# LiWentomng/OrientedRepPoints

Hardware: NVIDIA H100
Metric: 1024x1024 tiles/sec (higher is better)
Workload: dtype f16x3

## Files before the change

include/orp_b200.h:

```cpp
#ifndef ORP_B200_H_
#define ORP_B200_H_

#include <stdint.h>

#ifdef __cplusplus
extern "C" {
#endif

#define ORP_OK 0
#define ORP_EINVAL (-1)
#define ORP_ECUDA (-2)
#define ORP_ENOGPU (-3)
#define ORP_EOVERFLOW (-4)

const char *orp_last_error(void);
int orp_version(void);
int orp_compiled_sm(void);
int64_t orp_launch_count(void);
void orp_reset_launch_count(void);


#define ORP_NMS_EXACT64 0
#define ORP_NMS_COMPAT32 1

#define ORP_UNION_NAN_KEEPS 0
#define ORP_UNION_GUARD 1
#define ORP_UNION_NAN_SUPPRESSES 2
#define ORP_UNION_NAN_SUPPRESSES_ALL 3

#define ORP_ORDER_INDEX_ASC 0
#define ORP_ORDER_SCORE_DESC 1

int orp_rnms(const float *dets, const int32_t *segments, int n, double iou_thr, int iou_mode,
             int union_mode, int order, int64_t *keep_out, int32_t *num_out, void *stream);

int orp_poly_nms_host(int *keep_out, int *num_out, const float *polys_host, int polys_num,
                      int polys_dim, float nms_overlap_thresh, int device_id);

typedef struct {
    int64_t pairs_total;
    int64_t pairs_aabb;
    int64_t pairs_clipped;
    int64_t pairs_fp64;
    int64_t edges;
    int64_t suppressing;
    int32_t overflow;
    int32_t rounds;
    int32_t n;
} orp_nms_stats;
int orp_rnms_last_stats(orp_nms_stats *out);

typedef struct {
    int32_t lazy;
    int32_t R;
    int32_t seg_limit;
    int32_t sweep_bits;
    int32_t no_sync;
    int32_t flags_out;
    int32_t union_mode, order, n;
    int64_t cap_first;
    int64_t cap_final;
    int32_t attempts;
} orp_rnms_plan;
int orp_rnms_last_plan(orp_rnms_plan *out);

void orp_set_timing(int on);
int orp_rnms_last_sweep_ms(float *ms);
int orp_tc_timing_collect(float *total_ms, int *launches, double *flops);
typedef struct {
    int BN;
    int stages;
    int grid;
    int num_tiles;
    int n_tiles_n;
    int ksplit;
    int nprob;
    int Cout, Cout_padded;
    int split;
    int deform;
    int out_f32;
    int stem;
    int relu;
    int bias;
    int residual;
    int tma_epi, ncat, dcat, res_mma, b_resident, epi_merge, epi_bufs, gn_fused;
    int BW[5], BH[5], BI[5];
} orp_tc_plan;
int orp_tc_last_plan(orp_tc_plan *out);


int orp_poly_overlaps_host(float *overlaps, const float *boxes, const float *query_boxes, int n,
                           int k, int device_id);
int orp_poly_overlaps(const float *boxes5, int n, const float *query5, int k, float *out,
                      void *stream);

int orp_quad_iou_matrix(const float *quads_a, int n, const float *quads_b, int k, int iou_mode,
                        int union_mode, float *out, void *stream);

int orp_iou_poly_f64_pairs(const double *p8, const double *q8, int n, double *out, void *stream);

int orp_convex_iou(const float *pts18, int n, const float *quads8, int k, float *out, void *stream);

int orp_box_iou_rotated(const float *boxes1, int n, const float *boxes2, int m, float *out,
                        void *stream);


int orp_minarearect(const float *pts, int n, float *out, int32_t *hull_map, float scale,
                    const float *center, void *stream);


int orp_head_postprocess(int nlevels, const float *const *cls, const float *const *ref, const int *H,
                         const int *W, const int *stride, int B, int num_cls, int nms_pre, float score_thr,
                         double iou_thr, int max_per_img, const float *scale_factor, float *dets_out,
                         int64_t *labels_out, int32_t *counts_out, void *stream);
int orp_pack_detections(const float *dets, const int64_t *labels, const int32_t *counts, int B, int max_per_img,
                        float *packed_out, void *stream);
int orp_dcn_offsets_multi(int nprob, const float *const *pts, float *const *off, const long long *numel,
                          float gradient_mul, const float *base18, void *stream);


int orp_conv2d_f32(const float *x, int N, int H, int W, int Cin, const float *w, int Cout, int KH, int KW,
                   int stride, int pad, const float *bias, const float *residual, int relu, float *y,
                   double *gn_stats, int groups, void *stream);

int orp_deform_conv2d_f32(const float *x, int N, int H, int W, int Cin, const float *offset, const float *mask,
                          const float *w, int Cout, int KH, int KW, int stride, int pad, int dilation,
                          const float *bias, int relu, float *y, void *stream);

int orp_gn_apply_f32(const float *x, int N, int H, int W, int C, const double *stats, int groups,
                     const float *gamma, const float *beta, float eps, int relu, const float *up_src, float *y,
                     void *stream);

int orp_maxpool3x3s2_f32(const float *x, int N, int H, int W, int C, float *y, void *stream);


typedef struct {
    const void *x;
    int N, H, W;
    void *out;
    const void *residual_bf16;
    const float *residual_f32;
    const float *offset;
    double *gn_stats;
    const float *mask;
} orp_tc_problem;

int orp_conv2d_bf16(int nprob, const orp_tc_problem *probs, const void *w, int Cout, int Cout_padded,
                    int KH, int KW, int Cin, int stride, int pad, const float *bias, int relu, int out_f32,
                    int deform, void *stream);

int orp_conv2d_f16x3(int nprob, const orp_tc_problem *probs, const void *w_split, int Cout, int Cout_padded,
                     int KH, int KW, int Cin, int stride, int pad, const float *bias, int wscale_log2, int relu,
                     int out_f32, int deform, void *stream);
int orp_conv2d_tc_splitk(const orp_tc_problem *prob, const void *w, int Cout, int Cout_padded, int KH, int KW, int Cin,
                         int stride, int pad, const float *bias, int f16x3, int wscale_log2, int relu, int ksplit,
                         float *workspace, void *stream);
int orp_tc_plan_conv(int nprob, const orp_tc_problem *probs, const void *w, int Cout, int Cout_padded, int KH, int KW,
                     int Cin, int stride, int pad, const float *bias, int wscale_log2, int relu, int out_f32, int deform,
                     int split, int stem, int ksplit, int sms, orp_tc_plan *out);
int orp_f16x3_overflow_count(unsigned int *count, int reset);
int orp_stem_s2d_u8_f16x3(const uint8_t *img_hwc, int N, int H, int W, const float *mean, const float *std, int to_rgb,
                          void *out, void *stream);
int orp_stem_s2d_u8_padded_f16x3(const uint8_t *img_hwc, int N, int H, int W, const float *mean, const float *std, int to_rgb,
                                 const int32_t *valid_hw, void *out, void *stream);
int orp_stem_s2d_f16x3(const float *img_nchw, int N, int H, int W, void *out, void *stream);
int orp_stem_conv_s2d_f16x3(const void *x_s2d, int N, int H, int W, const void *w_split, const float *bias,
                            int wscale_log2, int relu, void *out, void *stream);
int orp_maxpool3x3s2_f16x3(const void *x, int N, int H, int W, int C, void *y, void *stream);
int orp_gn_stats_f16x3(const void *x, int N, int HW, int C, int groups, double *stats, void *stream);
int orp_split_from_f32(const float *x, long long pixels, int C, void *y_split, void *stream);
int orp_split_to_f32(const void *x_split, long long pixels, int C, float *y, void *stream);
int orp_transpose_f32(const float *x, int N, int R, int Cc, float *y, void *stream);
int orp_nchw_f32_to_split(const float *x, int N, int C, int HW, void *y_split, void *stream);

int orp_stem_im2col_bf16(const float *img_nchw, int N, int H, int W, void *out, void *stream);
int orp_stem_s2d_bf16(const float *img_nchw, int N, int H, int W, void *out, void *stream);
int orp_stem_conv_s2d_bf16(const void *x_s2d, int N, int H, int W, const void *w256, const float *bias, int relu,
                           void *out, void *stream);
int orp_stem_s2d_u8_bf16(const uint8_t *img_hwc, int N, int H, int W, const float *mean, const float *std, int to_rgb,
                         void *out, void *stream);
int orp_stem_s2d_u8_padded_bf16(const uint8_t *img_hwc, int N, int H, int W, const float *mean, const float *std, int to_rgb,
                                const int32_t *valid_hw, void *out, void *stream);
int orp_maxpool3x3s2_bf16(const void *x, int N, int H, int W, int C, void *y, void *stream);
int orp_gn_stats_bf16(const void *x, int N, int HW, int C, int groups, double *stats, void *stream);
typedef struct orp_gn_problem {
    const void *x;
    int N, H, W;
    const double *stats;
    const void *up_src;
    void *y;
} orp_gn_problem;
int orp_gn_apply_bf16_multi(int nprob, const orp_gn_problem *probs, int C, int groups, const float *gamma,
                            const float *beta, float eps, int relu, void *stream);
int orp_gn_apply_f16x3_multi(int nprob, const orp_gn_problem *probs, int C, int groups, const float *gamma,
                             const float *beta, float eps, int relu, void *stream);

int orp_split_tiles_u8(const uint8_t *img_hwc, int H, int W, int C, const int32_t *origins, int ntiles, int subsize,
                       uint8_t *out, void *stream);

int orp_resize_u8(const uint8_t *src, int N, int H, int W, int C, uint8_t *dst, int Hd, int Wd, int Hp, int Wp, int flip,
                  const int32_t *xtab, const int32_t *ytab, void *stream);


int orp_layernorm_bf16(const void *x, int B, int H, int W, int C, const float *gamma, const float *beta, float eps,
                       int Hp, int Wp, void *y, void *stream);
int orp_window_attention_bf16(const void *qkv, int B, int H, int W, int Hp, int Wp, int C, int heads, int shift,
                              const float *bias_table, float scale, void *out, void *stream);
int orp_patch_embed_rows_bf16(const float *img_nchw, int B, int H, int W, void *out, void *stream);
int orp_patch_embed_rows_u8_bf16(const uint8_t *img_hwc, int B, int H, int W, const float *mean, const float *stdinv, int to_rgb,
                                 void *out, void *stream);
int orp_patch_embed_rows_u8_padded_bf16(const uint8_t *img_hwc, int B, int H, int W, const float *mean, const float *stdinv,
                                        int to_rgb, const int32_t *valid_hw, void *out, void *stream);
int orp_patch_merge_gather_bf16(const void *x, int B, int H, int W, int C, void *y, void *stream);
int orp_subsample2_bf16(const void *x, int B, int H, int W, int C, void *y, void *stream);
int orp_layernorm_f16x3(const void *x, int B, int H, int W, int C, const float *gamma, const float *beta, float eps,
                        int Hp, int Wp, void *y, void *stream);
int orp_window_attention_f16x3(const void *qkv, int B, int H, int W, int Hp, int Wp, int C, int heads, int shift,
                               const float *bias_table, float scale, void *out, void *stream);
int orp_patch_embed_rows_f16x3(const float *img_nchw, int B, int H, int W, void *out, void *stream);
int orp_patch_embed_rows_u8_f16x3(const uint8_t *img_hwc, int B, int H, int W, const float *mean, const float *stdinv, int to_rgb,
                                  void *out, void *stream);
int orp_patch_embed_rows_u8_padded_f16x3(const uint8_t *img_hwc, int B, int H, int W, const float *mean, const float *stdinv,
                                         int to_rgb, const int32_t *valid_hw, void *out, void *stream);
int orp_patch_merge_gather_f16x3(const void *x, int B, int H, int W, int C, void *y, void *stream);
int orp_subsample2_f16x3(const void *x, int B, int H, int W, int C, void *y, void *stream);

#ifdef __cplusplus
}
#endif
#endif
```

orientedreppoints_b200/_lib.py:

```python
import ctypes
import os

_HERE = os.path.dirname(os.path.abspath(__file__))
LIB_PATH = os.path.join(_HERE, "lib", "liborp_b200.so")

ORP_NMS_EXACT64, ORP_NMS_COMPAT32 = 0, 1
ORP_UNION_NAN_KEEPS, ORP_UNION_GUARD, ORP_UNION_NAN_SUPPRESSES, ORP_UNION_NAN_SUPPRESSES_ALL = 0, 1, 2, 3
ORP_ORDER_INDEX_ASC, ORP_ORDER_SCORE_DESC = 0, 1

_vp = ctypes.c_void_p
_i = ctypes.c_int
_f = ctypes.c_float
_d = ctypes.c_double


class NmsStats(ctypes.Structure):
    _fields_ = [("pairs_total", ctypes.c_int64), ("pairs_aabb", ctypes.c_int64),
                ("pairs_clipped", ctypes.c_int64), ("pairs_fp64", ctypes.c_int64),
                ("edges", ctypes.c_int64), ("suppressing", ctypes.c_int64), ("overflow", ctypes.c_int32),
                ("rounds", ctypes.c_int32), ("n", ctypes.c_int32)]

    def as_dict(self):
        return {k: int(getattr(self, k)) for k, _ in self._fields_}


class RnmsPlan(ctypes.Structure):
    _fields_ = [(k, ctypes.c_int32) for k in ("lazy", "R", "seg_limit", "sweep_bits", "no_sync", "flags_out", "union_mode",
                                              "order", "n")] + \
              [("cap_first", ctypes.c_int64), ("cap_final", ctypes.c_int64), ("attempts", ctypes.c_int32)]

    def as_dict(self):
        return {k: int(getattr(self, k)) for k, _ in self._fields_}


class TcProblem(ctypes.Structure):
    _fields_ = [("x", _vp), ("N", _i), ("H", _i), ("W", _i), ("out", _vp), ("residual_bf16", _vp),
                ("residual_f32", _vp), ("offset", _vp), ("gn_stats", _vp), ("mask", _vp)]


class TcPlan(ctypes.Structure):
    _fields_ = [(k, _i) for k in ("BN", "stages", "grid", "num_tiles", "n_tiles_n", "ksplit", "nprob", "Cout", "Cout_padded",
                                  "split", "deform", "out_f32", "stem", "relu", "bias", "residual", "tma_epi", "ncat", "dcat",
                                  "res_mma", "b_resident", "epi_merge", "epi_bufs", "gn_fused")] + \
              [(k, _i * 5) for k in ("BW", "BH", "BI")]

    def as_dict(self):
        d = {k: getattr(self, k) for k, _ in self._fields_}
        for k in ("BW", "BH", "BI"):
            d[k] = list(d[k])[:self.nprob]
        return d


class GnProblem(ctypes.Structure):
    _fields_ = [("x", _vp), ("N", _i), ("H", _i), ("W", _i), ("stats", _vp), ("up_src", _vp), ("y", _vp)]


SIGNATURES = {
    "orp_last_error": (ctypes.c_char_p, []),
    "orp_version": (_i, []),
    "orp_compiled_sm": (_i, []),
    "orp_launch_count": (ctypes.c_int64, []),
    "orp_reset_launch_count": (None, []),
    "orp_rnms": (_i, [_vp, _vp, _i, _d, _i, _i, _i, _vp, _vp, _vp]),
    "orp_poly_nms_host": (_i, [_vp, _vp, _vp, _i, _i, _f, _i]),
    "orp_rnms_last_stats": (_i, [ctypes.POINTER(NmsStats)]),
    "orp_rnms_last_plan": (_i, [ctypes.POINTER(RnmsPlan)]),
    "orp_set_timing": (None, [_i]),
    "orp_rnms_last_sweep_ms": (_i, [ctypes.POINTER(ctypes.c_float)]),
    "orp_tc_timing_collect": (_i, [ctypes.POINTER(ctypes.c_float), ctypes.POINTER(_i), ctypes.POINTER(_d)]),
    "orp_tc_last_plan": (_i, [ctypes.POINTER(TcPlan)]),
    "orp_poly_overlaps_host": (_i, [_vp, _vp, _vp, _i, _i, _i]),
    "orp_poly_overlaps": (_i, [_vp, _i, _vp, _i, _vp, _vp]),
    "orp_quad_iou_matrix": (_i, [_vp, _i, _vp, _i, _i, _i, _vp, _vp]),
    "orp_iou_poly_f64_pairs": (_i, [_vp, _vp, _i, _vp, _vp]),
    "orp_box_iou_rotated": (_i, [_vp, _i, _vp, _i, _vp, _vp]),
    "orp_minarearect": (_i, [_vp, _i, _vp, _vp, _f, _vp, _vp]),
    "orp_head_postprocess": (_i, [_i, _vp, _vp, _vp, _vp, _vp, _i, _i, _i, _f, _d, _i, _vp, _vp, _vp, _vp, _vp]),
    "orp_pack_detections": (_i, [_vp, _vp, _vp, _i, _i, _vp, _vp]),
    "orp_dcn_offsets_multi": (_i, [_i, _vp, _vp, _vp, _f, _vp, _vp]),
    "orp_conv2d_f32": (_i, [_vp, _i, _i, _i, _i, _vp, _i, _i, _i, _i, _i, _vp, _vp, _i, _vp, _vp, _i, _vp]),
    "orp_deform_conv2d_f32": (_i, [_vp, _i, _i, _i, _i, _vp, _vp, _vp, _i, _i, _i, _i, _i, _i, _vp, _i, _vp, _vp]),
    "orp_gn_apply_f32": (_i, [_vp, _i, _i, _i, _i, _vp, _i, _vp, _vp, _f, _i, _vp, _vp, _vp]),
    "orp_maxpool3x3s2_f32": (_i, [_vp, _i, _i, _i, _i, _vp, _vp]),
    "orp_conv2d_bf16": (_i, [_i, ctypes.POINTER(TcProblem), _vp, _i, _i, _i, _i, _i, _i, _i, _vp, _i, _i, _i, _vp]),
    "orp_conv2d_f16x3": (_i, [_i, ctypes.POINTER(TcProblem), _vp, _i, _i, _i, _i, _i, _i, _i, _vp, _i, _i, _i, _i, _vp]),
    "orp_conv2d_tc_splitk": (_i, [ctypes.POINTER(TcProblem), _vp, _i, _i, _i, _i, _i, _i, _i, _vp, _i, _i, _i, _i, _vp, _vp]),
    "orp_tc_plan_conv": (_i, [_i, ctypes.POINTER(TcProblem), _vp, _i, _i, _i, _i, _i, _i, _i, _vp, _i, _i, _i, _i, _i, _i, _i, _i,
                              ctypes.POINTER(TcPlan)]),
    "orp_f16x3_overflow_count": (_i, [ctypes.POINTER(ctypes.c_uint), _i]),
    "orp_stem_s2d_u8_f16x3": (_i, [_vp, _i, _i, _i, _vp, _vp, _i, _vp, _vp]),
    "orp_stem_s2d_f16x3": (_i, [_vp, _i, _i, _i, _vp, _vp]),
    "orp_stem_conv_s2d_f16x3": (_i, [_vp, _i, _i, _i, _vp, _vp, _i, _i, _vp, _vp]),
    "orp_maxpool3x3s2_f16x3": (_i, [_vp, _i, _i, _i, _i, _vp, _vp]),
    "orp_gn_stats_f16x3": (_i, [_vp, _i, _i, _i, _i, _vp, _vp]),
    "orp_gn_apply_f16x3_multi": (_i, [_i, _vp, _i, _i, _vp, _vp, _f, _i, _vp]),
    "orp_split_from_f32": (_i, [_vp, ctypes.c_longlong, _i, _vp, _vp]),
    "orp_split_to_f32": (_i, [_vp, ctypes.c_longlong, _i, _vp, _vp]),
    "orp_transpose_f32": (_i, [_vp, _i, _i, _i, _vp, _vp]),
    "orp_nchw_f32_to_split": (_i, [_vp, _i, _i, _i, _vp, _vp]),
    "orp_layernorm_bf16": (_i, [_vp, _i, _i, _i, _i, _vp, _vp, _f, _i, _i, _vp, _vp]),
    "orp_window_attention_bf16": (_i, [_vp, _i, _i, _i, _i, _i, _i, _i, _i, _vp, _f, _vp, _vp]),
    "orp_patch_embed_rows_bf16": (_i, [_vp, _i, _i, _i, _vp, _vp]),
    "orp_patch_embed_rows_u8_bf16": (_i, [_vp, _i, _i, _i, _vp, _vp, _i, _vp, _vp]),
    "orp_patch_merge_gather_bf16": (_i, [_vp, _i, _i, _i, _i, _vp, _vp]),
    "orp_subsample2_bf16": (_i, [_vp, _i, _i, _i, _i, _vp, _vp]),
    "orp_layernorm_f16x3": (_i, [_vp, _i, _i, _i, _i, _vp, _vp, _f, _i, _i, _vp, _vp]),
    "orp_window_attention_f16x3": (_i, [_vp, _i, _i, _i, _i, _i, _i, _i, _i, _vp, _f, _vp, _vp]),
    "orp_patch_embed_rows_f16x3": (_i, [_vp, _i, _i, _i, _vp, _vp]),
    "orp_patch_embed_rows_u8_f16x3": (_i, [_vp, _i, _i, _i, _vp, _vp, _i, _vp, _vp]),
    "orp_patch_merge_gather_f16x3": (_i, [_vp, _i, _i, _i, _i, _vp, _vp]),
    "orp_subsample2_f16x3": (_i, [_vp, _i, _i, _i, _i, _vp, _vp]),
    "orp_stem_im2col_bf16": (_i, [_vp, _i, _i, _i, _vp, _vp]),
    "orp_stem_s2d_bf16": (_i, [_vp, _i, _i, _i, _vp, _vp]),
    "orp_convex_iou": (_i, [_vp, _i, _vp, _i, _vp, _vp]),
    "orp_split_tiles_u8": (_i, [_vp, _i, _i, _i, _vp, _i, _i, _vp, _vp]),
    "orp_resize_u8": (_i, [_vp, _i, _i, _i, _i, _vp, _i, _i, _i, _i, _i, _vp, _vp, _vp]),
    "orp_stem_s2d_u8_padded_bf16": (_i, [_vp, _i, _i, _i, _vp, _vp, _i, _vp, _vp, _vp]),
    "orp_stem_s2d_u8_padded_f16x3": (_i, [_vp, _i, _i, _i, _vp, _vp, _i, _vp, _vp, _vp]),
    "orp_patch_embed_rows_u8_padded_bf16": (_i, [_vp, _i, _i, _i, _vp, _vp, _i, _vp, _vp, _vp]),
    "orp_patch_embed_rows_u8_padded_f16x3": (_i, [_vp, _i, _i, _i, _vp, _vp, _i, _vp, _vp, _vp]),
    "orp_stem_s2d_u8_bf16": (_i, [_vp, _i, _i, _i, _vp, _vp, _i, _vp, _vp]),
    "orp_stem_conv_s2d_bf16": (_i, [_vp, _i, _i, _i, _vp, _vp, _i, _vp, _vp]),
    "orp_maxpool3x3s2_bf16": (_i, [_vp, _i, _i, _i, _i, _vp, _vp]),
    "orp_gn_stats_bf16": (_i, [_vp, _i, _i, _i, _i, _vp, _vp]),
    "orp_gn_apply_bf16_multi": (_i, [_i, _vp, _i, _i, _vp, _vp, _f, _i, _vp]),
}

_LIB = None


class OrpError(RuntimeError):
    pass


def lib():
    global _LIB
    if _LIB is None:
        if not os.path.exists(LIB_PATH):
            raise OrpError(
                "liborp_b200.so not found at %s - build it with `python -m orientedreppoints_b200.build` "
                "(there is no CPU or PyTorch fallback for this path)" % LIB_PATH)
        l = ctypes.CDLL(LIB_PATH)
        for name, (res, args) in SIGNATURES.items():
            fn = getattr(l, name)
            fn.restype = res
            fn.argtypes = args
        _LIB = l
    return _LIB


def check(rc, what=""):
    if rc != 0:
        msg = lib().orp_last_error()
        raise OrpError("%s failed (%d): %s" % (what, rc, msg.decode() if msg else ""))


def launch_count():
    return int(lib().orp_launch_count())


def reset_launch_count():
    lib().orp_reset_launch_count()


def last_nms_stats():
    s = NmsStats()
    check(lib().orp_rnms_last_stats(ctypes.byref(s)), "orp_rnms_last_stats")
    return s.as_dict()


def rnms_last_plan():
    p = RnmsPlan()
    check(lib().orp_rnms_last_plan(ctypes.byref(p)), "orp_rnms_last_plan")
    return p.as_dict()


def set_timing(on):
    lib().orp_set_timing(1 if on else 0)


def last_sweep_ms():
    v = ctypes.c_float(0)
    check(lib().orp_rnms_last_sweep_ms(ctypes.byref(v)), "orp_rnms_last_sweep_ms")
    return float(v.value)


def tc_timing_collect():
    ms, n, fl = ctypes.c_float(0), ctypes.c_int(0), ctypes.c_double(0)
    check(lib().orp_tc_timing_collect(ctypes.byref(ms), ctypes.byref(n), ctypes.byref(fl)), "orp_tc_timing_collect")
    return float(ms.value), int(n.value), float(fl.value)


def tc_last_plan():
    p = TcPlan()
    check(lib().orp_tc_last_plan(ctypes.byref(p)), "orp_tc_last_plan")
    return p.as_dict()


def tc_plan_for(problems, cout, cout_p, kh, kw, cin, stride, pad, *, bias=False, relu=0, out_f32=False, deform=False,
                split=False, residual=0, gn=False, stem=0, ksplit=1, sms=132):
    ph = 256
    arr = (TcProblem * len(problems))()
    for q, (n, h, w) in zip(arr, problems):
        q.x, q.N, q.H, q.W, q.out = ph, n, h, w, ph
        q.residual_bf16 = ph if residual == 1 else None
        q.residual_f32 = ph if residual == 2 else None
        q.offset = ph if deform else None
        q.gn_stats = ph if gn else None
    p = TcPlan()
    check(lib().orp_tc_plan_conv(len(problems), arr, ph, cout, cout_p, kh, kw, cin, stride, pad, ph if bias else None, 0,
                                 int(relu), int(out_f32), int(deform), int(split), stem, ksplit, sms, ctypes.byref(p)),
          "orp_tc_plan_conv")
    return p.as_dict()


def current_stream_ptr():
    import torch
    return ctypes.c_void_p(torch.cuda.current_stream().cuda_stream)


def ptr(t):
    return ctypes.c_void_p(0 if t is None else t.data_ptr())
```

orientedreppoints_b200/csrc/dense_tc.cu:

```cuda
#include <cuda.h>
#include <cuda_bf16.h>
#include <cuda_fp16.h>

#include <cstdlib>
#include <mutex>
#include <type_traits>

#include "common.cuh"
#include "wgmma.cuh"

namespace orp {
namespace {

constexpr int kMaxProb = 5;
constexpr int kStagesMax = 6;
constexpr int kBM = 128;
constexpr int kBK = 64;
constexpr int kABytes = kBM * kBK * 2;

struct FastDiv {
    uint32_t mul, shr, d;
    __host__ void set(uint32_t div)
    {
        d = div;
        uint32_t l = 0;
        while ((1ull << l) < div) ++l;
        shr = l;
        mul = (uint32_t)(((1ull << 32) * ((1ull << l) - div)) / div + 1);
    }
    __device__ __forceinline__ uint32_t div(uint32_t n) const { return (__umulhi(n, mul) + n) >> shr; }
    __device__ __forceinline__ void divmod(uint32_t n, uint32_t &q, uint32_t &r) const { q = div(n); r = n - q * d; }
};

struct Problem {
    int N, H, W, Ho, Wo;
    FastDiv fd_tw, fd_th;
    int BW, BH, BI;
    int lbw, lbh;
    int tiles_w, tiles_h, tiles_i, tile_start;
    void *out;
    const __nv_bfloat16 *res;
    const float *res32;
    const __nv_bfloat16 *x;
    const float *offset;
    const float *mask;
    double *gn_stats;
};

struct alignas(64) TcParams {
    CUtensorMap tmA[kMaxProb];
    CUtensorMap tmB;
    CUtensorMap tmOut[kMaxProb];
    CUtensorMap tmRes[kMaxProb];
    CUtensorMap tmI;
    Problem prob[kMaxProb];
    int tma_epi, epi_bufs;
    int epi_merge;
    int ncat;
    int ksplit;
    FastDiv fd_ks;
    long long ks_stride;
    int b_resident;
    int res_mma;
    int gn_fused;
    int dcat;
    int split;
    float oscale;
    unsigned int *ovf;
    int nprob, num_m_tiles, n_tiles_n, num_tiles;
    FastDiv fd_ntn;
    int KH, KW, Cin, cin_blocks, stride, pad, Cout, relu;
    int s2d_stem;
    const float *bias;
};

__device__ __forceinline__ uint32_t smem_u32(const void *p) { return (uint32_t)__cvta_generic_to_shared(p); }

__device__ __forceinline__ void mbar_init(uint64_t *bar, uint32_t count)
{
    asm volatile("mbarrier.init.shared::cta.b64 [%0], %1;" ::"r"(smem_u32(bar)), "r"(count));
}
__device__ __forceinline__ void mbar_expect_tx(uint64_t *bar, uint32_t bytes)
{
    asm volatile("mbarrier.arrive.expect_tx.shared::cta.b64 _, [%0], %1;" ::"r"(smem_u32(bar)), "r"(bytes) : "memory");
}
__device__ __forceinline__ void mbar_arrive(uint64_t *bar)
{
    asm volatile("mbarrier.arrive.shared::cta.b64 _, [%0];" ::"r"(smem_u32(bar)) : "memory");
}
__device__ __forceinline__ void mbar_wait(uint64_t *bar, uint32_t parity)
{
    asm volatile(
        "{\n\t"
        ".reg .pred p;\n\t"
        "WAIT_LOOP:\n\t"
        "mbarrier.try_wait.parity.shared::cta.b64 p, [%0], %1;\n\t"
        "@p bra WAIT_DONE;\n\t"
        "bra WAIT_LOOP;\n\t"
        "WAIT_DONE:\n\t"
        "}" ::"r"(smem_u32(bar)), "r"(parity) : "memory");
}
__device__ __forceinline__ bool elect_one()
{
    uint32_t pred = 0;
    asm volatile(
        "{\n\t"
        ".reg .pred P1;\n\t"
        "elect.sync _|P1, %1;\n\t"
        "selp.b32 %0, 1, 0, P1;\n\t"
        "}" : "=r"(pred) : "r"(0xffffffffu));
    return pred != 0;
}
__device__ __forceinline__ void tma_load_4d(void *smem, const CUtensorMap *tm, uint64_t *bar, int c0, int c1, int c2, int c3)
{
    asm volatile(
        "cp.async.bulk.tensor.4d.shared::cluster.global.mbarrier::complete_tx::bytes [%0], [%1, {%3, %4, %5, %6}], [%2];"
        ::"r"(smem_u32(smem)), "l"(tm), "r"(smem_u32(bar)), "r"(c0), "r"(c1), "r"(c2), "r"(c3) : "memory");
}
__device__ __forceinline__ void tma_load_5d(void *smem, const CUtensorMap *tm, uint64_t *bar, int c0, int c1, int c2, int c3, int c4)
{
    asm volatile(
        "cp.async.bulk.tensor.5d.shared::cluster.global.mbarrier::complete_tx::bytes [%0], [%1, {%3, %4, %5, %6, %7}], [%2];"
        ::"r"(smem_u32(smem)), "l"(tm), "r"(smem_u32(bar)), "r"(c0), "r"(c1), "r"(c2), "r"(c3), "r"(c4) : "memory");
}
__device__ __forceinline__ void tma_load_2d(void *smem, const CUtensorMap *tm, uint64_t *bar, int c0, int c1)
{
    asm volatile(
        "cp.async.bulk.tensor.2d.shared::cluster.global.mbarrier::complete_tx::bytes [%0], [%1, {%3, %4}], [%2];"
        ::"r"(smem_u32(smem)), "l"(tm), "r"(smem_u32(bar)), "r"(c0), "r"(c1) : "memory");
}
__device__ __forceinline__ uint64_t make_desc_sw128(uint32_t smem_addr)
{
    uint64_t d = 0;
    d |= (uint64_t)((smem_addr >> 4) & 0x3FFF);
    d |= (uint64_t)1 << 16;
    d |= (uint64_t)(1024 >> 4) << 32;
    d |= (uint64_t)1 << 62;
    return d;
}
__device__ __forceinline__ uint4 lds128(uint32_t addr)
{
    uint4 v;
    asm volatile("ld.shared.v4.b32 {%0, %1, %2, %3}, [%4];" : "=r"(v.x), "=r"(v.y), "=r"(v.z), "=r"(v.w) : "r"(addr) : "memory");
    return v;
}
__device__ __forceinline__ void sts128(uint32_t addr, const uint4 &v)
{
    asm volatile("st.shared.v4.b32 [%0], {%1, %2, %3, %4};" ::"r"(addr), "r"(v.x), "r"(v.y), "r"(v.z), "r"(v.w) : "memory");
}
template <int ID, int N>
__device__ __forceinline__ void named_bar()
{
    asm volatile("bar.sync %0, %1;" ::"n"(ID), "n"(N) : "memory");
}
__device__ __forceinline__ void acc_ld32(uint32_t addr, uint32_t (&r)[32])
{
#pragma unroll
    for (int j = 0; j < 8; ++j) {
        const uint4 v = lds128(addr + (uint32_t)j * 16u);
        r[4 * j] = v.x; r[4 * j + 1] = v.y; r[4 * j + 2] = v.z; r[4 * j + 3] = v.w;
    }
}

__device__ __forceinline__ float2 ffma2_rn(float2 a, float2 b, float2 c) { return make_float2(__fmaf_rn(a.x, b.x, c.x), __fmaf_rn(a.y, b.y, c.y)); }
__device__ __forceinline__ float2 fadd2_rn(float2 a, float2 b) { return make_float2(__fadd_rn(a.x, b.x), __fadd_rn(a.y, b.y)); }

__device__ __forceinline__ float act_fn(float v, int act)
{
    if (act == 1) return fmaxf(v, 0.f);
    if (act == 2) return 0.5f * v * (1.0f + erff(v * 0.70710678118654752f));
    return v;
}

struct Ring {
    int stage = 0;
    uint32_t phase = 0;
    int n;
    __device__ explicit Ring(int n_) : n(n_) {}
    __device__ void next() { if (++stage == n) { stage = 0; phase ^= 1; } }
};

struct KIter {
    int tap, term, cb = 0, phase = 0;
    int tap0, taps, cbn, mode;
    __device__ KIter(int taps_, int cbn_, int mode_, int tap0_ = 0) : tap0(tap0_), taps(taps_), cbn(cbn_), mode(mode_)
    {
        tap = tap0;
        term = (mode == 1) ? 1 : 0;
    }
    __device__ void next()
    {
        if (mode == 0) { if (++cb == cbn) { cb = 0; ++tap; } }
        else if (phase == 0) {
            if (++cb == cbn) { cb = 0; if (++term == 3) { term = 1; if (++tap == taps) { tap = tap0; term = 0; phase = 1; } } }
        } else { if (++cb == cbn) { cb = 0; ++tap; } }
    }
};

__device__ __forceinline__ int ksplit_of(const TcParams &P, int tile)
{
    if (P.ksplit <= 1) return 0;
    uint32_t q, r;
    P.fd_ks.divmod((uint32_t)tile, q, r);
    return (int)r;
}

__device__ __forceinline__ void decode_tile(const TcParams &P, int tile, int &pi, int &wb, int &hb, int &ib, int &nt)
{
    uint32_t mt_u, nt_u;
    if (P.ksplit > 1) tile = (int)P.fd_ks.div((uint32_t)tile);
    P.fd_ntn.divmod((uint32_t)tile, mt_u, nt_u);
    nt = (int)nt_u;
    const int mt = (int)mt_u;
    pi = 0;
#pragma unroll
    for (int k = 1; k < kMaxProb; ++k)
        if (k < P.nprob && mt >= P.prob[k].tile_start) pi = k;
    const Problem &pr = P.prob[pi];
    const int local = mt - pr.tile_start;
    uint32_t rest, wb_u, ib_u, hb_u;
    pr.fd_tw.divmod((uint32_t)local, rest, wb_u);
    pr.fd_th.divmod(rest, ib_u, hb_u);
    wb = (int)wb_u; hb = (int)hb_u; ib = (int)ib_u;
}

struct IdentBlock { unsigned short v[64 * 64]; };
constexpr IdentBlock make_ident()
{
    IdentBlock b{};
    for (int i = 0; i < 64; ++i) b.v[i * 64 + i] = 0x3F80;
    return b;
}
__device__ IdentBlock g_ident = make_ident();
struct IdentBlocks16 { unsigned short v[16][64 * 64]; };
constexpr IdentBlocks16 make_ident16()
{
    IdentBlocks16 b{};
    for (int s = 0; s < 16; ++s)
        for (int i = 0; i < 64; ++i) b.v[s][i * 64 + i] = (unsigned short)((15 + s) << 10);
    return b;
}
__device__ IdentBlocks16 g_ident16 = make_ident16();
__device__ unsigned int g_f16_overflow = 0;

constexpr int kConsumers = 256;
constexpr int kDP = 256;
constexpr int kDItems = 1024 / kDP;
constexpr int kDRound = kDItems / 2;
constexpr int kAccPitch = 68;
constexpr int kAccBytes = 128 * kAccPitch * 4;

__host__ __device__ constexpr int stage_bytes(int BN, bool cat, bool b_resident)
{
    return cat ? (b_resident ? 2 * kABytes : 2 * kABytes + 2 * BN * kBK * 2) : (b_resident ? kABytes : kABytes + BN * kBK * 2);
}
constexpr int dyn_smem_bytes(int stage_b, int stages, int extra) { return 1024 + kAccBytes + stages * stage_b + extra; }

template <int BN, int R>
__device__ __forceinline__ void stage_acc(const float (&acc)[R], int pass, bool ncat, float *s_acc, int row0, int col0)
{
    constexpr int kGroups = (BN < 64 ? BN : 64) / 8;
#pragma unroll
    for (int p = 0; p < (BN + 63) / 64; ++p) {
        if (p != pass) continue;
#pragma unroll
        for (int i = 0; i < kGroups; ++i) {
            const int g = p * 8 + i;
            float2 a = make_float2(acc[4 * g], acc[4 * g + 1]), b = make_float2(acc[4 * g + 2], acc[4 * g + 3]);
            if constexpr (R >= BN) {
                if (ncat) {
                    a.x += acc[BN / 2 + 4 * g]; a.y += acc[BN / 2 + 4 * g + 1];
                    b.x += acc[BN / 2 + 4 * g + 2]; b.y += acc[BN / 2 + 4 * g + 3];
                }
            }
            *reinterpret_cast<float2 *>(s_acc + row0 * kAccPitch + i * 8 + col0) = a;
            *reinterpret_cast<float2 *>(s_acc + (row0 + 8) * kAccPitch + i * 8 + col0) = b;
        }
    }
}

constexpr int kWalkK = 0;
constexpr int kWalkNcat = 1;
constexpr int kWalkDcat = 2;
constexpr int kWalkKRes = 3;

template <int NG, bool BF16, int R, int G = 0>
__device__ __forceinline__ void wgmma_cols64(float (&acc)[R], uint64_t da, uint64_t db, uint32_t accumulate)
{
    wgmma_n<64, BF16>(acc_view<32 * G, 32>(acc), da, db + (uint64_t)(G * 512), accumulate);
    if constexpr (G + 1 < NG) wgmma_cols64<NG, BF16, R, G + 1>(acc, da, db, accumulate);
}

constexpr int kProducerRegs = 40;
constexpr int kConsumerRegs = 232;

template <int BN, bool OUT_F32, bool DEFORM, bool SPLIT, int WALK>
__global__ void __launch_bounds__(DEFORM ? kConsumers + kDP : kConsumers + 128, 1)
conv_tc_kernel(const __grid_constant__ TcParams P, int stages)
{
    static_assert(WALK != kWalkNcat || (SPLIT && !DEFORM && !OUT_F32 && BN >= 64 && BN <= 128), "ncat: f16x3 TMA-epilogue layers, BN 64..128");
    static_assert(!DEFORM || (WALK == kWalkDcat) == SPLIT, "deformable: dcat exactly in f16x3");
    static_assert(DEFORM || WALK != kWalkDcat, "dcat is the deformable walk");
    static_assert(WALK != kWalkKRes || (!DEFORM && !OUT_F32 && BN >= 64), "residual K blocks: TMA-epilogue layers");
    constexpr bool kBF16 = !SPLIT;
    constexpr int kWTerms = SPLIT ? 2 : 1;
    constexpr bool kCat = WALK == kWalkNcat || WALK == kWalkDcat;
    constexpr int kKMode = (SPLIT && !kCat) ? 1 : 0;
    static_assert(kConsumers + 128 == 384 && 2 * 128 * kConsumerRegs + 128 * kProducerRegs <= 65536, "register split");
    constexpr int kEpiThreads = kConsumers;
    constexpr int kWG = 2;
    constexpr int kAccN = (WALK == kWalkNcat) ? 2 * BN : BN;
    extern __shared__ __align__(1024) uint8_t smem_raw[];
    uint8_t *smem = reinterpret_cast<uint8_t *>((reinterpret_cast<uintptr_t>(smem_raw) + 1023) & ~uintptr_t(1023));
    float *s_acc = reinterpret_cast<float *>(smem);
    smem += kAccBytes;
    constexpr int kBBytes = BN * kBK * 2;
    const int kStageBytes = stage_bytes(BN, kCat, P.b_resident);
    const int kblocks_all = P.KH * P.KW * P.cin_blocks * kWTerms;
    uint8_t *ident = smem;
    if (P.res_mma) smem += 8192;
    uint8_t *bres = smem;
    if (P.b_resident) smem += (size_t)kblocks_all * kBBytes;
    constexpr int HC = BN < 64 ? BN : 64;
    constexpr int kPitch = HC * 2 + 16;
    uint8_t *stage_out = smem + (size_t)stages * kStageBytes;
    __shared__ uint64_t bars[2 * kStagesMax];
    __shared__ __align__(16) float s_bias[256];
    __shared__ uint64_t bres_bar;
    uint64_t *full = bars;
    uint64_t *empty = bars + kStagesMax;

    const int warp = threadIdx.x >> 5, lane = threadIdx.x & 31;

    if (warp == kConsumers / 32 && elect_one()) {
        if (!DEFORM) {
#pragma unroll 1
            for (int p = 0; p < P.nprob; ++p)
                asm volatile("prefetch.tensormap [%0];" ::"l"(&P.tmA[p]) : "memory");
        }
        asm volatile("prefetch.tensormap [%0];" ::"l"(&P.tmB) : "memory");
    }
    if (warp == 0) {
        if (elect_one()) {
            for (int s = 0; s < stages; ++s) {
                mbar_init(&full[s], DEFORM ? 1 + kDP / 32 : 1);
                mbar_init(&empty[s], kConsumers / 128);
            }
            mbar_init(&bres_bar, 1);
            asm volatile("fence.mbarrier_init.release.cluster;" ::: "memory");
        }
        __syncwarp();
    }
    __syncthreads();
    const int taps_per = (P.KH * P.KW) / (P.ksplit > 1 ? P.ksplit : 1);
    const int kblocks = taps_per * P.cin_blocks * (kKMode ? 3 : 1);
    asm volatile("griddepcontrol.launch_dependents;" ::: "memory");
    asm volatile("griddepcontrol.wait;" ::: "memory");

    if (warp < kConsumers / 32) {
        if constexpr (!DEFORM) setmaxnreg_inc<kConsumerRegs>();
        const int cw = warp >> 2;
        const uint32_t a_off = (uint32_t)cw * 8192u;
        const bool leader = (threadIdx.x & 127) == 0;
        float acc[kAccN / 2];
        Ring r(stages);
        const int q = warp & 3, wg = warp >> 2;
        const int et = threadIdx.x, nthr = kEpiThreads;
        const int bar_a = 1, bar_b = 3;
        const int ch0 = wg, chs = kWG;
        const int frow = cw * 64 + (warp & 3) * 16 + (lane >> 2), fcol = 2 * (lane & 3);
        const uint32_t s_acc_u = smem_u32(s_acc);
        auto bar_sync = [](int id, int n) { asm volatile("bar.sync %0, %1;" ::"r"(id), "r"(n) : "memory"); };
        int ob = 0;
        int bias_nt = -1;
        if ((P.b_resident || P.res_mma) && (int)blockIdx.x < P.num_tiles) mbar_wait(&bres_bar, 0);
        for (int tile = blockIdx.x; tile < P.num_tiles; tile += gridDim.x) {
            int res_groups = 0;
            if constexpr (WALK == kWalkKRes) {
                const int nt = tile - (int)P.fd_ntn.div((uint32_t)tile) * P.n_tiles_n;
                for (int g = 0; g < BN / 64 && nt * BN + g * 64 < P.Cout; ++g) ++res_groups;
            }
            const int tap_lo = ksplit_of(P, tile) * taps_per;
            KIter it(tap_lo + taps_per, P.cin_blocks, kKMode, tap_lo);
            int held = -1;
            auto release = [&](int next) {
                if (held >= 0 && leader) mbar_arrive(&empty[held]);
                held = next;
            };
            for (int kb = 0; kb < kblocks; ++kb, it.next()) {
                mbar_wait(&full[r.stage], r.phase);
                const uint32_t sa = smem_u32(smem + (size_t)r.stage * kStageBytes);
                const uint64_t da = make_desc_sw128(sa + a_off);
                const int slab = (it.tap * P.cin_blocks + it.cb) * kWTerms + (it.term == 2 ? 1 : 0);
                wgmma_fence();
                if constexpr (WALK == kWalkNcat) {
                    const uint32_t sb = P.b_resident ? smem_u32(bres + (size_t)slab * kBBytes) : sa + 2 * kABytes;
                    const uint64_t dl = make_desc_sw128(sa + kABytes + a_off);
                    const uint64_t dbh = make_desc_sw128(sb), dbl = make_desc_sw128(sb + kBBytes);
#pragma unroll
                    for (int k = 0; k < kBK / 16; ++k) {
                        const uint32_t first = (kb | k) ? 1u : 0u;
                        wgmma_n<BN, kBF16>(acc_view<0, BN / 2>(acc), da + (uint64_t)(k * 2), dbh + (uint64_t)(k * 2), first);
                        wgmma_n<BN, kBF16>(acc_view<BN / 2, BN / 2>(acc), da + (uint64_t)(k * 2), dbl + (uint64_t)(k * 2), first);
                        wgmma_n<BN, kBF16>(acc_view<BN / 2, BN / 2>(acc), dl + (uint64_t)(k * 2), dbh + (uint64_t)(k * 2), 1u);
                    }
                } else if constexpr (WALK == kWalkDcat) {
                    const uint64_t dl = make_desc_sw128(sa + kABytes + a_off);
                    const uint64_t dbh = make_desc_sw128(sa + 2 * kABytes), dbl = make_desc_sw128(sa + 2 * kABytes + kBBytes);
#pragma unroll
                    for (int k = 0; k < kBK / 16; ++k) {
                        wgmma_n<BN, kBF16>(acc, dl + (uint64_t)(k * 2), dbh + (uint64_t)(k * 2), (kb | k) ? 1u : 0u);
                        wgmma_n<BN, kBF16>(acc, da + (uint64_t)(k * 2), dbl + (uint64_t)(k * 2), 1u);
                        wgmma_n<BN, kBF16>(acc, da + (uint64_t)(k * 2), dbh + (uint64_t)(k * 2), 1u);
                    }
                } else {
                    const uint64_t db = make_desc_sw128(P.b_resident ? smem_u32(bres + (size_t)slab * kBBytes) : sa + kABytes);
#pragma unroll
                    for (int k = 0; k < kBK / 16; ++k) {
                        if constexpr (WALK == kWalkKRes)
                            wgmma_cols64<BN / 64, kBF16>(acc, da + (uint64_t)(k * 2), db + (uint64_t)(k * 2), (kb | k) ? 1u : 0u);
                        else
                            wgmma_n<BN, kBF16>(acc, da + (uint64_t)(k * 2), db + (uint64_t)(k * 2), (kb | k) ? 1u : 0u);
                    }
                }
                wgmma_commit();
                wgmma_wait<1>();
                release(r.stage);
                r.next();
            }
            if constexpr (WALK == kWalkKRes) {
                wgmma_wait<0>();
                release(-1);
                auto res_group = [&](auto gc) {
                    constexpr int G = decltype(gc)::value;
                    if (G >= res_groups) return;
#pragma unroll 1
                    for (int t = 0; t < kWTerms; ++t) {
                        mbar_wait(&full[r.stage], r.phase);
                        const uint64_t da = make_desc_sw128(smem_u32(smem + (size_t)r.stage * kStageBytes) + a_off);
                        const uint64_t db = make_desc_sw128(smem_u32(ident));
                        wgmma_fence();
#pragma unroll
                        for (int k = 0; k < kBK / 16; ++k)
                            wgmma_n<64, kBF16>(acc_view<32 * G, 32>(acc), da + (uint64_t)(k * 2), db + (uint64_t)(k * 2), 1u);
                        wgmma_commit();
                        wgmma_wait<1>();
                        release(r.stage);
                        r.next();
                    }
                };
                res_group(std::integral_constant<int, 0>{});
                if constexpr (BN >= 128) res_group(std::integral_constant<int, 1>{});
                if constexpr (BN >= 256) {
                    res_group(std::integral_constant<int, 2>{});
                    res_group(std::integral_constant<int, 3>{});
                }
            }
            wgmma_wait<0>();
            wgmma_fence_acc(acc);
            release(-1);

            int pi, wb, hb, ib, nt;
            decode_tile(P, tile, pi, wb, hb, ib, nt);
            const Problem &pr = P.prob[pi];
            const int rrow = q * 32 + lane;
            auto row_pixel = [&](int r, size_t &pix) -> bool {
                const int iw = r & (pr.BW - 1), ih = (r >> pr.lbw) & (pr.BH - 1), ii = r >> (pr.lbw + pr.lbh);
                const int w = wb * pr.BW + iw, h = hb * pr.BH + ih, n = ib * pr.BI + ii;
                pix = ((size_t)n * pr.Ho + h) * pr.Wo + w;
                return (w < pr.Wo) && (h < pr.Ho) && (n < pr.N);
            };
            size_t pix;
            const bool valid = row_pixel(rrow, pix);
            if (OUT_F32) {
#pragma unroll 1
                for (int pass = 0; pass < BN / HC; ++pass) {
                bar_sync(bar_a, nthr);
                stage_acc<BN>(acc, pass, false, s_acc, frow, fcol);
                bar_sync(bar_a, nthr);
#pragma unroll 1
                for (int ch = wg; ch < HC / 32; ch += kWG) {
                    uint32_t v[32];
                    acc_ld32(s_acc_u + (uint32_t)(rrow * kAccPitch + ch * 32) * 4u, v);
                    const int c0 = nt * BN + pass * HC + ch * 32;
                    if (valid && c0 < P.Cout) {
                        float *op = reinterpret_cast<float *>(pr.out) + pix * P.Cout + c0;
                        const float *rp = pr.res32 ? pr.res32 + pix * P.Cout + c0 : nullptr;
                        if (P.ksplit > 1) {
                            float *sp = op + (long long)ksplit_of(P, tile) * P.ks_stride;
                            for (int j = 0; j < 32; ++j) {
                                if (c0 + j >= P.Cout) break;
                                sp[j] = __uint_as_float(v[j]) * P.oscale;
                            }
                        } else
                        for (int j = 0; j < 32; ++j) {
                            if (c0 + j >= P.Cout) break;
                            float f = __uint_as_float(v[j]) * P.oscale;
                            if (P.bias) f += P.bias[c0 + j];
                            if (pr.res && !P.split) f += __bfloat162float(pr.res[pix * P.Cout + c0 + j]);
                            if (rp) f += rp[j];
                            f = act_fn(f, P.relu);
                            op[j] = f;
                        }
                    }
                }
                }
            } else if (P.tma_epi) {
                const uint32_t slot = P.epi_merge ? 32768u : 16384u;
                const uint32_t obuf_u = smem_u32(stage_out);
                const uint32_t bias_u = smem_u32(s_bias);
                const bool io = (et == 0);
                constexpr int kPasses = BN / 64;
                const int oterms = (P.split && !P.epi_merge) ? 2 : 1;
                if (nt != bias_nt) {
                    bar_sync(bar_a, nthr);
                    for (int c = et; c < BN; c += nthr) s_bias[c] = (P.bias && nt * BN + c < P.Cout) ? P.bias[nt * BN + c] : 0.f;
                    bias_nt = nt;
                }
                float amax = 0.f;
#pragma unroll 1
                for (int pass = 0; pass < kPasses * oterms; ++pass) {
                    const int half = oterms == 2 ? (pass >> 1) : pass, oterm = oterms == 2 ? (pass & 1) : 0;
                    if (io) {
                        if (P.epi_bufs == 2) asm volatile("cp.async.bulk.wait_group.read 1;" ::: "memory");
                        else asm volatile("cp.async.bulk.wait_group.read 0;" ::: "memory");
                    }
                    bar_sync(bar_a, nthr);
                    if (oterm == 0) {
                        stage_acc<BN>(acc, half, P.ncat != 0, s_acc, frow, fcol);
                        bar_sync(bar_a, nthr);
                    }
                    float gn_s = 0.f, gn_q = 0.f;
                    const uint32_t orow = obuf_u + (uint32_t)ob * slot + (uint32_t)rrow * 128u;
#pragma unroll 1
                    for (int ch = ch0; ch < 2; ch += chs) {
                        const uint32_t arow = s_acc_u + (uint32_t)(rrow * kAccPitch + ch * 32) * 4u;
#pragma unroll
                        for (int j4 = 0; j4 < 4; ++j4) {
                            const int c16 = ch * 4 + j4;
                            const uint32_t sw = (uint32_t)(c16 ^ (rrow & 7)) << 4;
                            const uint4 a0 = lds128(arow + (uint32_t)j4 * 32u), a1 = lds128(arow + (uint32_t)j4 * 32u + 16u);
                            const float f0[8] = {__uint_as_float(a0.x), __uint_as_float(a0.y), __uint_as_float(a0.z), __uint_as_float(a0.w),
                                                 __uint_as_float(a1.x), __uint_as_float(a1.y), __uint_as_float(a1.z), __uint_as_float(a1.w)};
                            float f[8];
#pragma unroll
                            for (int j = 0; j < 8; ++j) f[j] = f0[j];
                            const uint32_t bb = bias_u + (uint32_t)(half * 64 + ch * 32 + j4 * 8) * 4u;
                            const uint4 b0 = lds128(bb), b1 = lds128(bb + 16u);
                            if (P.split) {
#pragma unroll
                                for (int j = 0; j < 8; ++j) f[j] *= P.oscale;
                            }
                            f[0] += __uint_as_float(b0.x); f[1] += __uint_as_float(b0.y);
                            f[2] += __uint_as_float(b0.z); f[3] += __uint_as_float(b0.w);
                            f[4] += __uint_as_float(b1.x); f[5] += __uint_as_float(b1.y);
                            f[6] += __uint_as_float(b1.z); f[7] += __uint_as_float(b1.w);
                            if (P.relu == 2) {
#pragma unroll
                                for (int j = 0; j < 8; ++j) f[j] = act_fn(f[j], 2);
                            }
                            uint32_t pk[4];
                            if (P.split) {
#pragma unroll
                                for (int j = 0; j < 8; ++j) {
                                    if (P.relu == 1) f[j] = fmaxf(f[j], 0.f);
                                    if (oterm == 0) amax = fmaxf(amax, fabsf(f[j]));
                                }
                                uint32_t pl[4];
#pragma unroll
                                for (int k = 0; k < 4; ++k) {
                                    const __half2 h2 = __floats2half2_rn(f[2 * k], f[2 * k + 1]);
                                    pk[k] = *reinterpret_cast<const uint32_t *>(&h2);
                                    if (P.epi_merge || oterm) {
                                        const float2 hf = __half22float2(h2);
                                        const __half2 l2 = __floats2half2_rn(f[2 * k] - hf.x, f[2 * k + 1] - hf.y);
                                        pl[k] = *reinterpret_cast<const uint32_t *>(&l2);
                                    }
                                }
                                if (P.epi_merge) sts128(orow + 16384u + sw, make_uint4(pl[0], pl[1], pl[2], pl[3]));
                                else if (oterm) { pk[0] = pl[0]; pk[1] = pl[1]; pk[2] = pl[2]; pk[3] = pl[3]; }
                            } else {
#pragma unroll
                                for (int k = 0; k < 4; ++k) {
                                    __nv_bfloat162 b2 = __floats2bfloat162_rn(f[2 * k], f[2 * k + 1]);
                                    if (P.relu == 1) b2 = __hmax2(b2, __floats2bfloat162_rn(0.f, 0.f));
                                    pk[k] = *reinterpret_cast<uint32_t *>(&b2);
                                }
                            }
                            sts128(orow + sw, make_uint4(pk[0], pk[1], pk[2], pk[3]));
                            if (P.gn_fused && oterm == 0) {
                                float gs = 0.f, gq = 0.f;
                                if (valid) {
#pragma unroll
                                    for (int j = 0; j < 8; ++j) { gs += f[j]; gq = fmaf(f[j], f[j], gq); }
                                }
#pragma unroll
                                for (int o = 16; o > 0; o >>= 1) {
                                    gs += __shfl_xor_sync(0xffffffffu, gs, o);
                                    gq += __shfl_xor_sync(0xffffffffu, gq, o);
                                }
                                if (lane == c16) { gn_s = gs; gn_q = gq; }
                            }
                        }
                    }
                    if (P.gn_fused && oterm == 0 && lane < 8 && (chs == 1 || (lane >> 2) == wg)) {
                        const int n_img = ib * pr.BI + ((q * 32) >> (pr.lbw + pr.lbh));
                        if (n_img < pr.N) {
                            double *st = pr.gn_stats + ((size_t)n_img * 32 + (size_t)(nt * BN + half * 64) / 8 + lane) * 2;
                            atomicAdd(st, (double)gn_s);
                            atomicAdd(st + 1, (double)gn_q);
                        }
                    }
                    asm volatile("fence.proxy.async.shared::cta;" ::: "memory");
                    bar_sync(bar_b, nthr);
                    if (io) {
                        asm volatile(
                            "cp.async.bulk.tensor.5d.global.shared::cta.bulk_group [%0, {%2, %3, %4, %5, %6}], [%1];"
                            ::"l"(&P.tmOut[pi]), "r"(obuf_u + (uint32_t)ob * slot), "r"(nt * BN + half * 64), "r"(oterm),
                              "r"(wb * pr.BW), "r"(hb * pr.BH), "r"(ib * pr.BI) : "memory");
                        if (P.epi_merge)
                            asm volatile(
                                "cp.async.bulk.tensor.5d.global.shared::cta.bulk_group [%0, {%2, %3, %4, %5, %6}], [%1];"
                                ::"l"(&P.tmOut[pi]), "r"(obuf_u + (uint32_t)ob * slot + 16384u), "r"(nt * BN + half * 64), "r"(1),
                                  "r"(wb * pr.BW), "r"(hb * pr.BH), "r"(ib * pr.BI) : "memory");
                        asm volatile("cp.async.bulk.commit_group;" ::: "memory");
                    }
                    if (++ob == P.epi_bufs) ob = 0;
                }
                if (P.split && valid && amax > 65504.f) atomicAdd(P.ovf, 1u);
            } else {
                const bool vec_ok = (P.Cout & 7) == 0;
                named_bar<1, kEpiThreads>();
                for (int c = et; c < BN; c += kEpiThreads) s_bias[c] = (P.bias && nt * BN + c < P.Cout) ? P.bias[nt * BN + c] : 0.f;
                named_bar<1, kEpiThreads>();
#pragma unroll 1
                for (int half = 0; half < BN / HC; ++half) {
                    const int cbase = nt * BN + half * HC;
                    constexpr int kChunksPerRow = HC / 8;
                    if (pr.res && vec_ok) {
                        for (int c = et; c < 128 * kChunksPerRow; c += kEpiThreads) {
                            const int r = c / kChunksPerRow, k16 = c - r * kChunksPerRow;
                            size_t rp;
                            const bool ok = row_pixel(r, rp) && (cbase + k16 * 8 < P.Cout);
                            const uint32_t dst = smem_u32(stage_out + (size_t)r * kPitch + k16 * 16);
                            if (ok) {
                                const __nv_bfloat16 *src = pr.res + rp * P.Cout + cbase + k16 * 8;
                                asm volatile("cp.async.cg.shared.global [%0], [%1], 16;" ::"r"(dst), "l"(src) : "memory");
                            }
                        }
                        asm volatile("cp.async.commit_group;" ::: "memory");
                    }
                    if (pr.res && vec_ok) asm volatile("cp.async.wait_group 0;" ::: "memory");
                    stage_acc<BN>(acc, half, false, s_acc, frow, fcol);
                    named_bar<1, kEpiThreads>();
#pragma unroll 1
                    for (int ch = wg; ch < HC / 32; ch += kWG) {
                        uint32_t v[32];
                        acc_ld32(s_acc_u + (uint32_t)(rrow * kAccPitch + ch * 32) * 4u, v);
                        const int c0 = cbase + ch * 32;
                        uint4 *sp = reinterpret_cast<uint4 *>(stage_out + (size_t)rrow * kPitch + ch * 64);
#pragma unroll
                        for (int j4 = 0; j4 < 4; ++j4) {
                            float f[8];
#pragma unroll
                            for (int j = 0; j < 8; ++j) f[j] = __uint_as_float(v[j4 * 8 + j]);
                            {
                                const float4 b0 = *reinterpret_cast<const float4 *>(&s_bias[half * HC + ch * 32 + j4 * 8]);
                                const float4 b1 = *reinterpret_cast<const float4 *>(&s_bias[half * HC + ch * 32 + j4 * 8 + 4]);
                                f[0] += b0.x; f[1] += b0.y; f[2] += b0.z; f[3] += b0.w;
                                f[4] += b1.x; f[5] += b1.y; f[6] += b1.z; f[7] += b1.w;
                            }
                            if (pr.res && !vec_ok && valid) {
                                for (int j = 0; j < 8; ++j)
                                    if (c0 + j4 * 8 + j < P.Cout) f[j] += __bfloat162float(pr.res[pix * P.Cout + c0 + j4 * 8 + j]);
                            }
                            if (pr.res && vec_ok && valid) {
                                const uint4 u = sp[j4];
                                const uint32_t uu[4] = {u.x, u.y, u.z, u.w};
#pragma unroll
                                for (int k = 0; k < 4; ++k) {
                                    const float2 r2 = __bfloat1622float2(*reinterpret_cast<const __nv_bfloat162 *>(&uu[k]));
                                    f[2 * k] += r2.x;
                                    f[2 * k + 1] += r2.y;
                                }
                            }
                            if (P.relu) {
#pragma unroll
                                for (int j = 0; j < 8; ++j) f[j] = act_fn(f[j], P.relu);
                            }
                            uint32_t pk[4];
#pragma unroll
                            for (int k = 0; k < 4; ++k) {
                                __nv_bfloat162 b2 = __floats2bfloat162_rn(f[2 * k], f[2 * k + 1]);
                                pk[k] = *reinterpret_cast<uint32_t *>(&b2);
                            }
                            sp[j4] = make_uint4(pk[0], pk[1], pk[2], pk[3]);
                        }
                    }
                    named_bar<1, kEpiThreads>();
                    for (int c = et; c < 128 * kChunksPerRow; c += kEpiThreads) {
                        const int r = c / kChunksPerRow, k16 = c - r * kChunksPerRow;
                        size_t rp;
                        if (row_pixel(r, rp) && (cbase + k16 * 8 < P.Cout)) {
                            const uint4 u = *reinterpret_cast<const uint4 *>(stage_out + (size_t)r * kPitch + k16 * 16);
                            __nv_bfloat16 *op = reinterpret_cast<__nv_bfloat16 *>(pr.out) + rp * P.Cout + cbase + k16 * 8;
                            if (vec_ok) {
                                *reinterpret_cast<uint4 *>(op) = u;
                            } else {
                                const __nv_bfloat16 *e8 = reinterpret_cast<const __nv_bfloat16 *>(&u);
                                for (int j = 0; j < 8; ++j) if (cbase + k16 * 8 + j < P.Cout) op[j] = e8[j];
                            }
                        }
                    }
                    named_bar<1, kEpiThreads>();
                }
            }
        }
        if (P.tma_epi && et == 0) asm volatile("cp.async.bulk.wait_group 0;" ::: "memory");
    } else if (!DEFORM) {
        setmaxnreg_dec<kProducerRegs>();
        if (warp == kConsumers / 32 && elect_one()) {
            Ring r(stages);
            if ((P.b_resident || P.res_mma) && (int)blockIdx.x < P.num_tiles) {
                const int nt0 = blockIdx.x % P.n_tiles_n;
                mbar_expect_tx(&bres_bar, (uint32_t)((P.b_resident ? kblocks_all * kBBytes : 0) + (P.res_mma ? 8192 : 0)));
                if (P.res_mma) tma_load_2d(ident, &P.tmI, &bres_bar, 0, 0);
                if (P.b_resident)
                    for (int kb = 0; kb < kblocks_all; ++kb)
                        tma_load_2d(bres + (size_t)kb * kBBytes, &P.tmB, &bres_bar, kb * kBK, nt0 * BN);
            }
            for (int tile = blockIdx.x; tile < P.num_tiles; tile += gridDim.x) {
                int pi, wb, hb, ib, nt;
                decode_tile(P, tile, pi, wb, hb, ib, nt);
                const Problem &pr = P.prob[pi];
                const int w0 = wb * pr.BW * P.stride - P.pad, h0 = hb * pr.BH * P.stride - P.pad, i0 = ib * pr.BI;
                const int tap_lo = ksplit_of(P, tile) * taps_per;
                KIter it(tap_lo + taps_per, P.cin_blocks, kKMode, tap_lo);
                for (int j = 0; j < kblocks; ++j, it.next()) {
                    const int kh = it.tap / P.KW, kw = it.tap - kh * P.KW;
                    mbar_wait(&empty[r.stage], r.phase ^ 1);
                    uint8_t *sa = smem + (size_t)r.stage * kStageBytes;
                    const int wblk = ((it.tap * P.cin_blocks + it.cb) * kWTerms) * kBK;
                    if constexpr (WALK == kWalkNcat) {
                        mbar_expect_tx(&full[r.stage], 2 * kABytes + (P.b_resident ? 0 : 2 * kBBytes));
                        tma_load_5d(sa, &P.tmA[pi], &full[r.stage], it.cb * kBK, 0, w0 + kw, h0 + kh, i0);
                        tma_load_5d(sa + kABytes, &P.tmA[pi], &full[r.stage], it.cb * kBK, 1, w0 + kw, h0 + kh, i0);
                        if (!P.b_resident) {
                            tma_load_2d(sa + 2 * kABytes, &P.tmB, &full[r.stage], wblk, nt * BN);
                            tma_load_2d(sa + 2 * kABytes + kBBytes, &P.tmB, &full[r.stage], wblk + kBK, nt * BN);
                        }
                    } else {
                        mbar_expect_tx(&full[r.stage], P.b_resident ? kABytes : kABytes + kBBytes);
                        tma_load_5d(sa, &P.tmA[pi], &full[r.stage], it.cb * kBK, it.term == 1 ? 1 : 0, w0 + kw, h0 + kh, i0);
                        if (!P.b_resident)
                            tma_load_2d(sa + kABytes, &P.tmB, &full[r.stage], wblk + (it.term == 2 ? kBK : 0), nt * BN);
                    }
                    r.next();
                }
                if constexpr (WALK == kWalkKRes) {
                    for (int g = 0; g < BN / 64 && nt * BN + g * 64 < P.Cout; ++g)
                        for (int t = 0; t < kWTerms; ++t) {
                            mbar_wait(&empty[r.stage], r.phase ^ 1);
                            mbar_expect_tx(&full[r.stage], kABytes);
                            tma_load_5d(smem + (size_t)r.stage * kStageBytes, &P.tmRes[pi], &full[r.stage], nt * BN + g * 64, t,
                                        wb * pr.BW, hb * pr.BH, ib * pr.BI);
                            r.next();
                        }
                }
            }
        }
    } else if (DEFORM) {
        __shared__ float4 s_w[2][128];
        __shared__ uint2 s_wh[2][128];
        __shared__ int4 s_o[2][128];
        const int pt = threadIdx.x - kConsumers;
        auto load_b = [&](int stage, int tap, int cb, int nt) {
            uint8_t *sb = smem + (size_t)stage * kStageBytes + (P.dcat ? 2 * kABytes : kABytes);
            const int wblk = (tap * P.cin_blocks + cb) * (P.split ? 2 : 1) * kBK;
            mbar_expect_tx(&full[stage], P.dcat ? 2 * kBBytes : kBBytes);
            tma_load_2d(sb, &P.tmB, &full[stage], wblk, nt * BN);
            if (P.dcat) tma_load_2d(sb + kBBytes, &P.tmB, &full[stage], wblk + kBK, nt * BN);
        };
        Ring r(stages);
        int tb = 0;
        for (int tile = blockIdx.x; tile < P.num_tiles; tile += gridDim.x) {
            int pi, wb, hb, ib, nt;
            decode_tile(P, tile, pi, wb, hb, ib, nt);
            const Problem &pr = P.prob[pi];
            bool valid = false;
            int w = 0, h = 0, n = 0;
            if (pt < 128) {
                const int iw = pt & (pr.BW - 1), ih = (pt >> pr.lbw) & (pr.BH - 1), ii = pt >> (pr.lbw + pr.lbh);
                w = wb * pr.BW + iw; h = hb * pr.BH + ih; n = ib * pr.BI + ii;
                valid = (w < pr.Wo) && (h < pr.Ho) && (n < pr.N);
            }
            const int taps = P.KH * P.KW;
            const size_t opix = ((size_t)(valid ? n : 0) * pr.Ho + (valid ? h : 0)) * pr.Wo + (valid ? w : 0);
            const float *offp = pr.offset + opix * (2 * taps);
            const float *mskp = pr.mask ? pr.mask + opix * taps : nullptr;
            const int cpp = P.Cin * (P.split ? 2 : 1);
            const int img0 = (valid ? n : 0) * pr.H * pr.W * cpp;
            for (int tap = 0; tap < taps; ++tap) {
                if (pt < 128) {
                    const int kh = tap / P.KW, kw = tap - kh * P.KW;
                    float4 wv = make_float4(0.f, 0.f, 0.f, 0.f);
                    int4 ov = make_int4(img0, img0, img0, img0);
                    if (valid) {
                        const float h_im = (float)(h * P.stride - P.pad + kh) + offp[2 * tap];
                        const float w_im = (float)(w * P.stride - P.pad + kw) + offp[2 * tap + 1];
                        if (h_im > -1.f && w_im > -1.f && h_im < (float)pr.H && w_im < (float)pr.W) {
                            const int h_low = (int)floorf(h_im), w_low = (int)floorf(w_im);
                            const int h_high = h_low + 1, w_high = w_low + 1;
                            const float lh = h_im - (float)h_low, lw = w_im - (float)w_low, hh = 1.f - lh, hw = 1.f - lw;
                            if (h_low >= 0 && w_low >= 0) { wv.x = hh * hw; ov.x = img0 + (h_low * pr.W + w_low) * cpp; }
                            if (h_low >= 0 && w_high <= pr.W - 1) { wv.y = hh * lw; ov.y = img0 + (h_low * pr.W + w_high) * cpp; }
                            if (h_high <= pr.H - 1 && w_low >= 0) { wv.z = lh * hw; ov.z = img0 + (h_high * pr.W + w_low) * cpp; }
                            if (h_high <= pr.H - 1 && w_high <= pr.W - 1) { wv.w = lh * lw; ov.w = img0 + (h_high * pr.W + w_high) * cpp; }
                            if (mskp) {
                                const float m = mskp[tap];
                                wv.x *= m; wv.y *= m; wv.z *= m; wv.w *= m;
                            }
                        }
                    }
                    s_w[tb][pt] = wv;
                    s_o[tb][pt] = ov;
                    if (P.split) {
                        const __half2 w01 = __floats2half2_rn(wv.x, wv.y), w23 = __floats2half2_rn(wv.z, wv.w);
                        s_wh[tb][pt] = make_uint2(*reinterpret_cast<const uint32_t *>(&w01), *reinterpret_cast<const uint32_t *>(&w23));
                    }
                }
                asm volatile("bar.sync 2, %0;" ::"n"(kDP) : "memory");
                for (int cb = 0; cb < P.cin_blocks; ++cb) {
                    if (!P.split) {
                        mbar_wait(&empty[r.stage], r.phase ^ 1);
                        if (pt == 0) load_b(r.stage, tap, cb, nt);
                        uint8_t *sa = smem + (size_t)r.stage * kStageBytes;
                        uint4 u[kDItems][4];
#pragma unroll
                        for (int it = 0; it < kDItems; ++it) {
                            const int item = pt + it * kDP, row = item >> 3, c16 = item & 7;
                            const int4 ov = s_o[tb][row];
                            const int co = cb * kBK + c16 * 8;
                            u[it][0] = *reinterpret_cast<const uint4 *>(pr.x + ov.x + co);
                            u[it][1] = *reinterpret_cast<const uint4 *>(pr.x + ov.y + co);
                            u[it][2] = *reinterpret_cast<const uint4 *>(pr.x + ov.z + co);
                            u[it][3] = *reinterpret_cast<const uint4 *>(pr.x + ov.w + co);
                        }
#pragma unroll
                        for (int it = 0; it < kDItems; ++it) {
                            const int item = pt + it * kDP, row = item >> 3, c16 = item & 7;
                            const float4 wv = s_w[tb][row];
                            const uint32_t *a1 = reinterpret_cast<const uint32_t *>(&u[it][0]);
                            const uint32_t *a2 = reinterpret_cast<const uint32_t *>(&u[it][1]);
                            const uint32_t *a3 = reinterpret_cast<const uint32_t *>(&u[it][2]);
                            const uint32_t *a4 = reinterpret_cast<const uint32_t *>(&u[it][3]);
                            uint32_t pk[4];
#pragma unroll
                            for (int k = 0; k < 4; ++k) {
                                const float2 f1 = __bfloat1622float2(*reinterpret_cast<const __nv_bfloat162 *>(&a1[k]));
                                const float2 f2 = __bfloat1622float2(*reinterpret_cast<const __nv_bfloat162 *>(&a2[k]));
                                const float2 f3 = __bfloat1622float2(*reinterpret_cast<const __nv_bfloat162 *>(&a3[k]));
                                const float2 f4 = __bfloat1622float2(*reinterpret_cast<const __nv_bfloat162 *>(&a4[k]));
                                const float vx = wv.x * f1.x + wv.y * f2.x + wv.z * f3.x + wv.w * f4.x;
                                const float vy = wv.x * f1.y + wv.y * f2.y + wv.z * f3.y + wv.w * f4.y;
                                __nv_bfloat162 b2 = __floats2bfloat162_rn(vx, vy);
                                pk[k] = *reinterpret_cast<uint32_t *>(&b2);
                            }
                            *reinterpret_cast<uint4 *>(sa + (size_t)row * 128 + ((c16 ^ (row & 7)) << 4)) = make_uint4(pk[0], pk[1], pk[2], pk[3]);
                        }
                        asm volatile("fence.proxy.async.shared::cta;" ::: "memory");
                        __syncwarp();
                        if ((pt & 31) == 0) mbar_arrive(&full[r.stage]);
                        r.next();
                    } else {
                        const __half *xh = reinterpret_cast<const __half *>(pr.x);
                        uint32_t phi[kDItems][4], plo[kDItems][4];
#pragma unroll
                        for (int i2 = 0; i2 < 2; ++i2) {
                            uint4 u[kDRound][4][2];
#pragma unroll
                            for (int i1 = 0; i1 < kDRound; ++i1) {
                                const int item = pt + (i2 * kDRound + i1) * kDP, row = item >> 3, c16 = item & 7;
                                const int4 ov = s_o[tb][row];
                                const int co = cb * kBK + c16 * 8;
                                const int oo[4] = {ov.x, ov.y, ov.z, ov.w};
#pragma unroll
                                for (int c = 0; c < 4; ++c) {
                                    u[i1][c][0] = *reinterpret_cast<const uint4 *>(xh + oo[c] + co);
                                    u[i1][c][1] = *reinterpret_cast<const uint4 *>(xh + oo[c] + P.Cin + co);
                                }
                            }
#pragma unroll
                            for (int i1 = 0; i1 < kDRound; ++i1) {
                                const int it = i2 * kDRound + i1, item = pt + it * kDP, row = item >> 3;
                                const float4 wv = s_w[tb][row];
                                const uint2 wh = s_wh[tb][row];
                                const float2 wc[4] = {make_float2(wv.x, wv.x), make_float2(wv.y, wv.y), make_float2(wv.z, wv.z), make_float2(wv.w, wv.w)};
                                const __half2 wl[4] = {__low2half2(*reinterpret_cast<const __half2 *>(&wh.x)), __high2half2(*reinterpret_cast<const __half2 *>(&wh.x)),
                                                       __low2half2(*reinterpret_cast<const __half2 *>(&wh.y)), __high2half2(*reinterpret_cast<const __half2 *>(&wh.y))};
#pragma unroll
                                for (int k = 0; k < 4; ++k) {
                                    float2 acc = make_float2(0.f, 0.f);
                                    __half2 accl = __float2half2_rn(0.f);
#pragma unroll
                                    for (int c = 0; c < 4; ++c) {
                                        const uint32_t uh = reinterpret_cast<const uint32_t *>(&u[i1][c][0])[k];
                                        const uint32_t ul = reinterpret_cast<const uint32_t *>(&u[i1][c][1])[k];
                                        acc = ffma2_rn(wc[c], __half22float2(*reinterpret_cast<const __half2 *>(&uh)), acc);
                                        accl = __hfma2(wl[c], *reinterpret_cast<const __half2 *>(&ul), accl);
                                    }
                                    acc = fadd2_rn(acc, __half22float2(accl));
                                    const __half2 h2 = __floats2half2_rn(acc.x, acc.y);
                                    const float2 hf = __half22float2(h2);
                                    const float2 rem = fadd2_rn(acc, make_float2(-hf.x, -hf.y));
                                    const __half2 l2 = __floats2half2_rn(rem.x, rem.y);
                                    phi[it][k] = *reinterpret_cast<const uint32_t *>(&h2);
                                    plo[it][k] = *reinterpret_cast<const uint32_t *>(&l2);
                                }
                            }
                        }
                        {
                            mbar_wait(&empty[r.stage], r.phase ^ 1);
                            if (pt == 0) load_b(r.stage, tap, cb, nt);
                            uint8_t *sa = smem + (size_t)r.stage * kStageBytes;
#pragma unroll
                            for (int it = 0; it < kDItems; ++it) {
                                const int item = pt + it * kDP, row = item >> 3, c16 = item & 7;
                                const size_t at = (size_t)row * 128 + ((c16 ^ (row & 7)) << 4);
                                *reinterpret_cast<uint4 *>(sa + at) = make_uint4(phi[it][0], phi[it][1], phi[it][2], phi[it][3]);
                                *reinterpret_cast<uint4 *>(sa + kABytes + at) = make_uint4(plo[it][0], plo[it][1], plo[it][2], plo[it][3]);
                            }
                            asm volatile("fence.proxy.async.shared::cta;" ::: "memory");
                            __syncwarp();
                            if ((pt & 31) == 0) mbar_arrive(&full[r.stage]);
                            r.next();
                        }
                    }
                }
                tb ^= 1;
            }
        }
    }
}

typedef CUresult (*EncodeTiledFn)(CUtensorMap *, CUtensorMapDataType, cuuint32_t, void *, const cuuint64_t *, const cuuint64_t *,
                                  const cuuint32_t *, const cuuint32_t *, CUtensorMapInterleave, CUtensorMapSwizzle,
                                  CUtensorMapL2promotion, CUtensorMapFloatOOBfill);

EncodeTiledFn encode_fn()
{
    static EncodeTiledFn fn = nullptr;
    static std::once_flag once;
    std::call_once(once, [] {
        void *p = nullptr;
        cudaDriverEntryPointQueryResult st;
        if (cudaGetDriverEntryPoint("cuTensorMapEncodeTiled", &p, cudaEnableDefault, &st) == cudaSuccess && st == cudaDriverEntryPointSuccess)
            fn = reinterpret_cast<EncodeTiledFn>(p);
    });
    return fn;
}

int pow2_floor(int v) { int p = 1; while (p * 2 <= v) p *= 2; return p; }

constexpr int kEvPool = 1024;
thread_local cudaEvent_t g_tc_ev[kEvPool][2];
thread_local int g_tc_ev_created = 0, g_tc_ev_used = 0;
thread_local double g_tc_flops = 0.0;
struct TcTrace { int nprob, N, H, W, Cin, Cout, K, stride, deform, BN, tiles, grid; double flops; };
thread_local TcTrace g_tc_trace[kEvPool];
thread_local orp_tc_plan g_tc_plan;
thread_local bool g_tc_plan_set = false;

constexpr int kSmemPerBlock = 227 * 1024;
constexpr int kStaticSmemPlain = 4096;
constexpr int kStaticSmemDeform = 14336;

struct ConvDesc {
    int nprob;
    const orp_tc_problem *probs;
    const void *w;
    int Cout, Cout_padded, KH, KW, Cin, stride, pad;
    const float *bias;
    int relu, out_f32, deform;
    int split;
    int wscale_log2;
    int stem;
    int ksplit;
};

struct ConvPlan {
    orp_tc_plan rep;
    Problem prob[kMaxProb];
    int num_m_tiles;
    int extra_bytes;
};

int check_conv(const ConvDesc &d)
{
    if (d.split && (d.wscale_log2 < 0 || d.wscale_log2 > 15)) return fail(ORP_EINVAL, "conv2d_f16x3: weight scale exponent must be in 0..15");
    if (d.nprob < 1 || d.nprob > kMaxProb || !d.probs || !d.w) return fail(ORP_EINVAL, "conv2d_tc: bad arguments");
    if (d.Cin % 8) return fail(ORP_EINVAL, "conv2d_tc: Cin must be a multiple of 8 (16-byte channel rows)");
    if (d.deform && (d.Cin % kBK)) return fail(ORP_EINVAL, "conv2d_tc: deformable conv needs Cin % 64 == 0");
    if (d.Cout_padded % 32 || d.Cout_padded < d.Cout) return fail(ORP_EINVAL, "conv2d_tc: padded Cout must be a multiple of 32");
    if (d.stride < 1 || d.stride > 256) return fail(ORP_EINVAL, "conv2d_tc: stride must be in 1..256");
    if (d.deform)
        for (int i = 0; i < d.nprob; ++i)
            if ((long long)d.probs[i].N * d.probs[i].H * d.probs[i].W * d.Cin * (d.split ? 2 : 1) >= (1LL << 31))
                return fail(ORP_EINVAL, "conv2d_tc: deformable input has 2^31 or more 16-bit elements (32-bit sample offsets)");
    const orp_tc_problem &q0 = d.probs[0];
    if (d.ksplit > 1 && (d.nprob != 1 || d.deform || d.stem || !d.out_f32 || (d.KH * d.KW) % d.ksplit || q0.residual_bf16 ||
                         q0.residual_f32 || d.bias || d.relu))
        return fail(ORP_EINVAL, "conv2d_tc: split-K serves one plain problem with an fp32 partial-sum output and taps % ksplit == 0");
    return ORP_OK;
}

int plan_conv(const ConvDesc &d, int sms, ConvPlan &pl)
{
    int rc = check_conv(d);
    if (rc) return rc;
    memset(&pl, 0, sizeof(pl));
    const int nprob = d.nprob, ksplit = d.ksplit, T = d.split ? 2 : 1;
    const orp_tc_problem *probs = d.probs;

    int BN = 256;
    if (d.Cout_padded % 256) BN = (d.Cout_padded % 128 == 0) ? 128 : (d.Cout_padded % 64 == 0) ? 64 : 32;
    {
        long long mtiles = 0;
        for (int i = 0; i < nprob; ++i) {
            const int ho = (probs[i].H + 2 * d.pad - (d.KH - 1) - 1) / d.stride + 1, wo = (probs[i].W + 2 * d.pad - (d.KW - 1) - 1) / d.stride + 1;
            mtiles += ((long long)probs[i].N * ho * wo + 127) / 128;
        }
        while (BN > 64 && mtiles * (d.Cout_padded / BN) * ksplit < 120) BN /= 2;
    }
    if (d.deform && BN > 128) BN = 128;
    const int cin_blocks = (d.Cin + kBK - 1) / kBK;
    const int n_tiles_n = d.Cout_padded / BN;
    int mt = 0;
    for (int i = 0; i < nprob; ++i) {
        const orp_tc_problem &q = probs[i];
        Problem &pr = pl.prob[i];
        pr.N = q.N; pr.H = q.H; pr.W = q.W;
        pr.Ho = (q.H + 2 * d.pad - (d.KH - 1) - 1) / d.stride + 1;
        pr.Wo = (q.W + 2 * d.pad - (d.KW - 1) - 1) / d.stride + 1;
        if (pr.Ho <= 0 || pr.Wo <= 0 || !q.x || !q.out) return fail(ORP_EINVAL, "conv2d_tc: bad problem");
        pr.BW = pow2_floor(pr.Wo < 128 ? pr.Wo : 128);
        if (d.stride * pr.BW > 256) pr.BW = pow2_floor(256 / d.stride);
        pr.BH = pow2_floor(pr.Ho < 128 / pr.BW ? pr.Ho : 128 / pr.BW);
        pr.BI = 128 / (pr.BW * pr.BH);
        pr.lbw = 0; while ((1 << pr.lbw) < pr.BW) ++pr.lbw;
        pr.lbh = 0; while ((1 << pr.lbh) < pr.BH) ++pr.lbh;
        pr.tiles_w = ceil_div(pr.Wo, pr.BW); pr.tiles_h = ceil_div(pr.Ho, pr.BH); pr.tiles_i = ceil_div(pr.N, pr.BI);
        pr.tile_start = mt;
        pr.fd_tw.set((uint32_t)pr.tiles_w); pr.fd_th.set((uint32_t)pr.tiles_h);
        mt += pr.tiles_w * pr.tiles_h * pr.tiles_i;
        if (d.deform && !q.offset) return fail(ORP_EINVAL, "conv2d_tc: deformable conv needs offsets");
    }
    const int num_tiles = mt * n_tiles_n * ksplit;
    bool any_res = false;
    for (int i = 0; i < nprob; ++i) any_res = any_res || (probs[i].residual_bf16 != nullptr);
    const int tma_epi = (!d.out_f32 && ((d.Cout % 64 == 0) || (d.split && d.Cout % 8 == 0)) && BN >= 64) ? 1 : 0;
    if (d.split && !d.out_f32 && !tma_epi) return fail(ORP_EINVAL, "conv2d_f16x3: 16-bit outputs need Cout % 8 == 0 and weights padded to a multiple of 64 rows");
    if (d.split && d.out_f32 && any_res) return fail(ORP_EINVAL, "conv2d_f16x3: fp32 outputs take an fp32 residual only");
    bool want_gn = false, gn_ok = tma_epi && d.Cout == 256 && !d.bias && !d.relu;
    for (int i = 0; i < nprob; ++i) {
        want_gn = want_gn || (probs[i].gn_stats != nullptr);
        if (pl.prob[i].BW * pl.prob[i].BH < 32) gn_ok = false;
    }
    const int gn_fused = (want_gn && gn_ok) ? 1 : 0;
    const bool mem_bound = any_res || (d.KH * d.KW * (d.Cin / kBK) <= 8);
    int epi_bufs = mem_bound ? 2 : 1;
    const int epi_merge = (d.split && tma_epi && (mem_bound || d.stem == 2)) ? 1 : 0;
    const int dcat = (d.split && d.deform) ? 1 : 0;
    const int ncat = (d.split && tma_epi && BN <= 128 && !d.deform && !any_res) ? 1 : 0;
    const int res_mma = (tma_epi && any_res) ? 1 : 0;
    if (res_mma) {
        if (d.deform) return fail(ORP_EINVAL, "conv2d_tc: residual is not supported on the deformable path");
        for (int i = 0; i < nprob; ++i)
            if (!probs[i].residual_bf16) return fail(ORP_EINVAL, "conv2d_tc: residual must be given for every problem or none");
    }
    const int slab_bytes = d.KH * d.KW * T * cin_blocks * BN * kBK * 2;
    int b_resident = (!d.deform && ksplit == 1 && slab_bytes <= 72 * 1024) ? 1 : 0;
    int grid = num_tiles < sms ? num_tiles : sms;
    if (b_resident && grid >= n_tiles_n) grid -= grid % n_tiles_n;
    else if (b_resident) b_resident = 0;
    int stage_b = 0, extra = 0, stages = 0;
    for (;;) {
        stage_b = stage_bytes(BN, ncat || dcat, b_resident);
        const int hc = BN < 64 ? BN : 64;
        int staging = d.out_f32 ? 0 : 128 * (hc * 2 + 16);
        if (tma_epi) staging = epi_bufs * (epi_merge ? 32768 : 16384);
        extra = (res_mma ? 8192 : 0) + (b_resident ? slab_bytes : 0) + staging;
        stages = (kSmemPerBlock - (d.deform ? kStaticSmemDeform : kStaticSmemPlain) - dyn_smem_bytes(stage_b, 0, extra)) / stage_b;
        if (stages >= 3) break;
        if (epi_bufs == 2) { epi_bufs = 1; continue; }
        if (b_resident) { b_resident = 0; continue; }
        if (stages >= 2) break;
        return fail(ORP_EINVAL, "conv2d_tc: shared-memory budget cannot hold two main-loop stages");
    }
    if (stages > kStagesMax) stages = kStagesMax;
    if (d.deform && stages > 3) stages = 3;

    pl.num_m_tiles = mt;
    pl.extra_bytes = extra;
    orp_tc_plan &r = pl.rep;
    r.BN = BN; r.stages = stages; r.grid = grid; r.num_tiles = num_tiles; r.n_tiles_n = n_tiles_n;
    r.ksplit = ksplit; r.nprob = nprob; r.Cout = d.Cout; r.Cout_padded = d.Cout_padded;
    r.split = d.split ? 1 : 0; r.deform = d.deform ? 1 : 0; r.out_f32 = d.out_f32 ? 1 : 0; r.stem = d.stem; r.relu = d.relu;
    r.bias = d.bias ? 1 : 0;
    for (int i = 0; i < nprob; ++i) {
        if (probs[i].residual_bf16) r.residual = 1;
        else if (probs[i].residual_f32) r.residual = 2;
        r.BW[i] = pl.prob[i].BW; r.BH[i] = pl.prob[i].BH; r.BI[i] = pl.prob[i].BI;
    }
    r.tma_epi = tma_epi; r.ncat = ncat; r.dcat = dcat; r.res_mma = res_mma; r.b_resident = b_resident;
    r.epi_merge = epi_merge; r.epi_bufs = epi_bufs; r.gn_fused = gn_fused;
    return ORP_OK;
}

int make_params(const ConvDesc &d, const ConvPlan &pl, TcParams &P)
{
    memset(&P, 0, sizeof(P));
    P.nprob = d.nprob; P.KH = d.KH; P.KW = d.KW; P.Cin = d.Cin; P.cin_blocks = (d.Cin + kBK - 1) / kBK;
    P.stride = d.stride; P.pad = d.pad;
    P.Cout = d.Cout; P.relu = d.relu; P.bias = d.bias; P.s2d_stem = (d.stem == 2) ? 1 : 0;
    P.split = d.split ? 1 : 0;
    P.oscale = d.split ? ldexpf(1.f, -d.wscale_log2) : 1.f;
    {
        void *ovf = nullptr;
        ORP_CUDA(cudaGetSymbolAddress(&ovf, g_f16_overflow));
        P.ovf = static_cast<unsigned int *>(ovf);
    }
    P.n_tiles_n = pl.rep.n_tiles_n;
    P.fd_ntn.set((uint32_t)P.n_tiles_n);
    for (int i = 0; i < d.nprob; ++i) {
        const orp_tc_problem &q = d.probs[i];
        Problem &pr = P.prob[i];
        pr = pl.prob[i];
        pr.out = q.out; pr.res = static_cast<const __nv_bfloat16 *>(q.residual_bf16); pr.res32 = q.residual_f32;
        pr.x = static_cast<const __nv_bfloat16 *>(q.x); pr.offset = q.offset; pr.gn_stats = q.gn_stats; pr.mask = q.mask;
    }
    P.num_m_tiles = pl.num_m_tiles;
    P.num_tiles = pl.rep.num_tiles;
    P.ksplit = d.ksplit;
    P.fd_ks.set((uint32_t)d.ksplit);
    P.ks_stride = (long long)P.prob[0].N * P.prob[0].Ho * P.prob[0].Wo * d.Cout;
    P.tma_epi = pl.rep.tma_epi; P.epi_bufs = pl.rep.epi_bufs; P.epi_merge = pl.rep.epi_merge; P.ncat = pl.rep.ncat;
    P.b_resident = pl.rep.b_resident; P.res_mma = pl.rep.res_mma; P.gn_fused = pl.rep.gn_fused; P.dcat = pl.rep.dcat;
    return ORP_OK;
}

int encode_maps(const ConvDesc &d, const ConvPlan &pl, TcParams &P)
{
    EncodeTiledFn enc = encode_fn();
    if (!enc) return fail(ORP_ECUDA, "conv2d_tc: cuTensorMapEncodeTiled unavailable");
    const CUtensorMapDataType dt16 = d.split ? CU_TENSOR_MAP_DATA_TYPE_FLOAT16 : CU_TENSOR_MAP_DATA_TYPE_BFLOAT16;
    const int T = d.split ? 2 : 1, Cin = d.Cin, Cout = d.Cout, stride = d.stride;
    if (!d.deform) {
        for (int i = 0; i < d.nprob; ++i) {
            const orp_tc_problem &q = d.probs[i];
            const Problem &pr = P.prob[i];
            cuuint64_t gdim[5] = {(cuuint64_t)Cin, (cuuint64_t)T, (cuuint64_t)q.W, (cuuint64_t)q.H, (cuuint64_t)q.N};
            cuuint64_t gstr[4] = {(cuuint64_t)Cin * 2, (cuuint64_t)Cin * 2 * T, (cuuint64_t)q.W * Cin * 2 * T,
                                  (cuuint64_t)q.H * q.W * Cin * 2 * T};
            if (d.stem == 2) {
                gstr[0] = (cuuint64_t)q.N * q.H * (q.W + 3) * 32;
                gstr[1] = 32;
                gstr[2] = (cuuint64_t)(q.W + 3) * 32;
                gstr[3] = (cuuint64_t)q.H * (q.W + 3) * 32;
            }
            cuuint32_t box[5] = {(cuuint32_t)kBK, 1u, (cuuint32_t)(pr.BW * stride), (cuuint32_t)(pr.BH * stride), (cuuint32_t)pr.BI};
            cuuint32_t estr[5] = {1, 1, (cuuint32_t)stride, (cuuint32_t)stride, 1};
            CUresult r = enc(&P.tmA[i], dt16, 5, const_cast<void *>(q.x), gdim, gstr, box, estr,
                             CU_TENSOR_MAP_INTERLEAVE_NONE, CU_TENSOR_MAP_SWIZZLE_128B, CU_TENSOR_MAP_L2_PROMOTION_L2_128B,
                             CU_TENSOR_MAP_FLOAT_OOB_FILL_NONE);
            if (r != CUDA_SUCCESS) return fail(ORP_ECUDA, "conv2d_tc: cuTensorMapEncodeTiled(A) failed");
        }
    }
    {
        const cuuint64_t K = (cuuint64_t)d.KH * d.KW * T * P.cin_blocks * kBK;
        cuuint64_t gdim[2] = {K, (cuuint64_t)d.Cout_padded};
        cuuint64_t gstr[1] = {K * 2};
        cuuint32_t box[2] = {(cuuint32_t)kBK, (cuuint32_t)pl.rep.BN};
        cuuint32_t estr[2] = {1, 1};
        CUresult r = enc(&P.tmB, dt16, 2, const_cast<void *>(d.w), gdim, gstr, box, estr,
                         CU_TENSOR_MAP_INTERLEAVE_NONE, CU_TENSOR_MAP_SWIZZLE_128B, CU_TENSOR_MAP_L2_PROMOTION_L2_256B,
                         CU_TENSOR_MAP_FLOAT_OOB_FILL_NONE);
        if (r != CUDA_SUCCESS) return fail(ORP_ECUDA, "conv2d_tc: cuTensorMapEncodeTiled(B) failed");
    }
    if (P.res_mma) {
        void *ident_ptr = nullptr;
        if (d.split) {
            ORP_CUDA(cudaGetSymbolAddress(&ident_ptr, g_ident16));
            ident_ptr = static_cast<char *>(ident_ptr) + (size_t)d.wscale_log2 * 8192;
        } else {
            ORP_CUDA(cudaGetSymbolAddress(&ident_ptr, g_ident));
        }
        cuuint64_t gdim[2] = {64, 64};
        cuuint64_t gstr[1] = {128};
        cuuint32_t box[2] = {64, 64};
        cuuint32_t estr[2] = {1, 1};
        CUresult r = enc(&P.tmI, dt16, 2, ident_ptr, gdim, gstr, box, estr, CU_TENSOR_MAP_INTERLEAVE_NONE,
                         CU_TENSOR_MAP_SWIZZLE_128B, CU_TENSOR_MAP_L2_PROMOTION_NONE, CU_TENSOR_MAP_FLOAT_OOB_FILL_NONE);
        if (r != CUDA_SUCCESS) return fail(ORP_ECUDA, "conv2d_tc: cuTensorMapEncodeTiled(identity) failed");
    }
    if (P.tma_epi) {
        for (int i = 0; i < d.nprob; ++i) {
            const Problem &pr = P.prob[i];
            cuuint64_t gdim[5] = {(cuuint64_t)Cout, (cuuint64_t)T, (cuuint64_t)pr.Wo, (cuuint64_t)pr.Ho, (cuuint64_t)pr.N};
            cuuint64_t gstr[4] = {(cuuint64_t)Cout * 2, (cuuint64_t)Cout * 2 * T, (cuuint64_t)pr.Wo * Cout * 2 * T,
                                  (cuuint64_t)pr.Ho * pr.Wo * Cout * 2 * T};
            cuuint32_t box[5] = {64u, 1u, (cuuint32_t)pr.BW, (cuuint32_t)pr.BH, (cuuint32_t)pr.BI};
            cuuint32_t estr[5] = {1, 1, 1, 1, 1};
            CUresult r = enc(&P.tmOut[i], dt16, 5, pr.out, gdim, gstr, box, estr,
                             CU_TENSOR_MAP_INTERLEAVE_NONE, CU_TENSOR_MAP_SWIZZLE_128B, CU_TENSOR_MAP_L2_PROMOTION_NONE,
                             CU_TENSOR_MAP_FLOAT_OOB_FILL_NONE);
            if (r != CUDA_SUCCESS) return fail(ORP_ECUDA, "conv2d_tc: cuTensorMapEncodeTiled(out) failed");
            if (pr.res) {
                r = enc(&P.tmRes[i], dt16, 5, const_cast<__nv_bfloat16 *>(pr.res), gdim, gstr, box, estr,
                        CU_TENSOR_MAP_INTERLEAVE_NONE, CU_TENSOR_MAP_SWIZZLE_128B, CU_TENSOR_MAP_L2_PROMOTION_L2_128B,
                        CU_TENSOR_MAP_FLOAT_OOB_FILL_NONE);
                if (r != CUDA_SUCCESS) return fail(ORP_ECUDA, "conv2d_tc: cuTensorMapEncodeTiled(residual) failed");
            }
        }
    }
    return ORP_OK;
}

template <int BN, bool OUT_F32, bool DEFORM, bool SPLIT, int WALK>
int launch_tc(const TcParams &P, int stages, int grid, cudaStream_t st, int extra_bytes)
{
    constexpr bool kCat = WALK == kWalkNcat || WALK == kWalkDcat;
    const int smem = dyn_smem_bytes(stage_bytes(BN, kCat, P.b_resident), stages, extra_bytes);
    auto kern = conv_tc_kernel<BN, OUT_F32, DEFORM, SPLIT, WALK>;
    static int smem_max = -1;
    if (smem_max < 0) {
        cudaFuncAttributes fa;
        ORP_CUDA(cudaFuncGetAttributes(&fa, kern));
        ORP_CUDA(cudaFuncSetAttribute(kern, cudaFuncAttributeMaxDynamicSharedMemorySize, kSmemPerBlock - (int)fa.sharedSizeBytes));
        smem_max = kSmemPerBlock - (int)fa.sharedSizeBytes;
    }
    if (smem > smem_max) {
        char need[32];
        snprintf(need, sizeof(need), "%d", smem);
        return fail(ORP_EINVAL, "conv2d_tc: the plan's %s bytes of dynamic shared memory do not fit beside the static shared memory of %s",
                    need, __PRETTY_FUNCTION__);
    }
    int slot = -1;
    if (g_timing && g_tc_ev_used < kEvPool) {
        slot = g_tc_ev_used++;
        if (slot >= g_tc_ev_created) {
            ORP_CUDA(cudaEventCreate(&g_tc_ev[slot][0]));
            ORP_CUDA(cudaEventCreate(&g_tc_ev[slot][1]));
            g_tc_ev_created = slot + 1;
        }
        ORP_CUDA(cudaEventRecord(g_tc_ev[slot][0], st));
        double fl = 0;
        for (int i = 0; i < P.nprob; ++i)
            fl += 2.0 * P.prob[i].N * P.prob[i].Ho * P.prob[i].Wo * (double)P.Cout *
                  (P.s2d_stem ? 147.0 : (double)P.KH * P.KW * P.Cin);
        g_tc_flops += fl;
        g_tc_trace[slot] = TcTrace{P.nprob, P.prob[0].N, P.prob[0].H, P.prob[0].W, P.Cin, P.Cout, P.KH, P.stride, DEFORM ? 1 : 0,
                                   BN, P.num_tiles, grid, fl};
    }
    {
        cudaLaunchConfig_t cfg;
        memset(&cfg, 0, sizeof(cfg));
        cfg.gridDim = dim3((unsigned)grid);
        cfg.blockDim = dim3(DEFORM ? (unsigned)(kConsumers + kDP) : (unsigned)(kConsumers + 128));
        cfg.dynamicSmemBytes = smem;
        cfg.stream = st;
        cudaLaunchAttribute at[1];
        at[0].id = cudaLaunchAttributeProgrammaticStreamSerialization;
        at[0].val.programmaticStreamSerializationAllowed = 1;
        cfg.attrs = at;
        cfg.numAttrs = 1;
        ORP_CUDA(cudaLaunchKernelEx(&cfg, kern, P, stages));
    }
    ORP_LAUNCHED();
    if (slot >= 0) ORP_CUDA(cudaEventRecord(g_tc_ev[slot][1], st));
    return ORP_OK;
}

template <int BN, bool OUT_F32, bool DEFORM>
int launch_plan(const TcParams &P, int stages, int grid, cudaStream_t st, int extra_bytes)
{
    if constexpr (DEFORM) {
        if (P.dcat != P.split || P.ncat || P.res_mma) return fail(ORP_EINVAL, "conv2d_tc: deformable plan outside dcat == split");
        return P.split ? launch_tc<BN, OUT_F32, true, true, kWalkDcat>(P, stages, grid, st, extra_bytes)
                       : launch_tc<BN, OUT_F32, true, false, kWalkK>(P, stages, grid, st, extra_bytes);
    } else {
        if (P.ncat && P.res_mma) return fail(ORP_EINVAL, "conv2d_tc: ncat plan with a residual");
        if (P.ncat) {
            if constexpr (!OUT_F32 && BN >= 64 && BN <= 128) {
                if (P.split) return launch_tc<BN, false, false, true, kWalkNcat>(P, stages, grid, st, extra_bytes);
            }
            return fail(ORP_EINVAL, "conv2d_tc: ncat plan outside f16x3 TMA-epilogue layers with BN 64..128");
        }
        if (P.res_mma) {
            if constexpr (!OUT_F32 && BN >= 64)
                return P.split ? launch_tc<BN, false, false, true, kWalkKRes>(P, stages, grid, st, extra_bytes)
                               : launch_tc<BN, false, false, false, kWalkKRes>(P, stages, grid, st, extra_bytes);
            return fail(ORP_EINVAL, "conv2d_tc: residual K blocks outside TMA-epilogue layers with BN >= 64");
        }
        return P.split ? launch_tc<BN, OUT_F32, false, true, kWalkK>(P, stages, grid, st, extra_bytes)
                       : launch_tc<BN, OUT_F32, false, false, kWalkK>(P, stages, grid, st, extra_bytes);
    }
}

template <bool OUT_F32, bool DEFORM>
int launch_bn(const TcParams &P, const ConvPlan &pl, cudaStream_t st)
{
    const int s = pl.rep.stages, g = pl.rep.grid, e = pl.extra_bytes;
    switch (pl.rep.BN) {
    case 256:
        if constexpr (!DEFORM) return launch_plan<256, OUT_F32, false>(P, s, g, st, e);
        break;
    case 128: return launch_plan<128, OUT_F32, DEFORM>(P, s, g, st, e);
    case 64: return launch_plan<64, OUT_F32, DEFORM>(P, s, g, st, e);
    case 32: return launch_plan<32, OUT_F32, DEFORM>(P, s, g, st, e);
    }
    return fail(ORP_EINVAL, "conv2d_tc: unsupported tile width");
}

int device_sms(int &sms)
{
    static thread_local int dev_known = -1, sms_known = 0;
    int dev = 0;
    ORP_CUDA(cudaGetDevice(&dev));
    if (dev != dev_known) {
        ORP_CUDA(cudaDeviceGetAttribute(&sms_known, cudaDevAttrMultiProcessorCount, dev));
        dev_known = dev;
    }
    sms = sms_known;
    return ORP_OK;
}

int conv2d_tc(const ConvDesc &d, void *stream)
{
    int rc = check_conv(d);
    if (rc) return rc;
    rc = ensure_device();
    if (rc) return rc;
    int sms = 0;
    rc = device_sms(sms);
    if (rc) return rc;
    ConvPlan pl;
    rc = plan_conv(d, sms, pl);
    if (rc) return rc;
    TcParams P;
    rc = make_params(d, pl, P);
    if (rc) return rc;
    rc = encode_maps(d, pl, P);
    if (rc) return rc;
    g_tc_plan = pl.rep;
    g_tc_plan_set = true;
    cudaStream_t st = static_cast<cudaStream_t>(stream);
    rc = d.out_f32 ? (d.deform ? launch_bn<true, true>(P, pl, st) : launch_bn<true, false>(P, pl, st))
                   : (d.deform ? launch_bn<false, true>(P, pl, st) : launch_bn<false, false>(P, pl, st));
    if (rc) return rc;
    bool want_gn = false;
    for (int i = 0; i < d.nprob; ++i) want_gn = want_gn || (d.probs[i].gn_stats != nullptr);
    if (want_gn && !P.gn_fused) {
        if (d.out_f32 || d.Cout != 256) return fail(ORP_EINVAL, "conv2d_tc: gn_stats needs a 16-bit output with 256 channels");
        for (int i = 0; i < d.nprob; ++i)
            if (d.probs[i].gn_stats) {
                int r2 = d.split ? orp_gn_stats_f16x3(P.prob[i].out, P.prob[i].N, P.prob[i].Ho * P.prob[i].Wo, 256, 32, d.probs[i].gn_stats, stream)
                                 : orp_gn_stats_bf16(P.prob[i].out, P.prob[i].N, P.prob[i].Ho * P.prob[i].Wo, 256, 32, d.probs[i].gn_stats, stream);
                if (r2) return r2;
            }
    }
    return ORP_OK;
}

int stem_desc(const void *x_s2d, int N, int H, int W, const void *w, const float *bias, int relu, void *out, int split,
              int wscale_log2, orp_tc_problem &q, ConvDesc &d)
{
    if (!x_s2d || !w || !out || N < 1 || H < 2 || W < 2 || (H & 1) || (W & 1))
        return fail(ORP_EINVAL, "stem_conv_s2d_%s: needs even H, W", split ? "f16x3" : "bf16");
    if (split && (wscale_log2 < 0 || wscale_log2 > 15)) return fail(ORP_EINVAL, "stem_conv_s2d_f16x3: weight scale exponent must be in 0..15");
    memset(&q, 0, sizeof(q));
    q.x = x_s2d;
    q.N = N; q.H = H / 2 + 3; q.W = W / 2; q.out = out;
    d = ConvDesc{1, &q, w, 64, 64, 4, 1, 64, 1, 0, bias, relu, 0, 0, split, split ? wscale_log2 : 0, 2, 1};
    return ORP_OK;
}

int splitk_desc(const orp_tc_problem *prob, const void *w, int Cout, int Cout_padded, int KH, int KW, int Cin, int stride, int pad,
                int f16x3, int wscale_log2, int ksplit, void *workspace, orp_tc_problem &q, ConvDesc &d, int &Ho, int &Wo)
{
    if (!prob || !w || !workspace || ksplit < 2 || (Cout % 8)) return fail(ORP_EINVAL, "conv2d_tc_splitk: bad arguments");
    if (f16x3 && (wscale_log2 < 0 || wscale_log2 > 15)) return fail(ORP_EINVAL, "conv2d_tc_splitk: weight scale exponent must be in 0..15");
    Ho = (prob->H + 2 * pad - (KH - 1) - 1) / stride + 1;
    Wo = (prob->W + 2 * pad - (KW - 1) - 1) / stride + 1;
    if (Ho <= 0 || Wo <= 0) return fail(ORP_EINVAL, "conv2d_tc_splitk: bad problem");
    q = *prob;
    q.out = workspace;
    q.gn_stats = nullptr;
    d = ConvDesc{1, &q, w, Cout, Cout_padded, KH, KW, Cin, stride, pad, nullptr, 0, 1, 0, f16x3 ? 1 : 0, wscale_log2, 0, ksplit};
    return ORP_OK;
}

__global__ void __launch_bounds__(256)
splitk_finish_kernel(const float *__restrict__ ws, int ksplit, size_t pixels, int C, const float *__restrict__ bias, int relu, int split,
                     void *__restrict__ out, unsigned int *ovf)
{
    const int c8 = C / 8;
    const size_t total = pixels * c8;
    for (size_t i = blockIdx.x * (size_t)blockDim.x + threadIdx.x; i < total; i += (size_t)gridDim.x * blockDim.x) {
        const size_t pix = i / c8;
        const int c = (int)(i - pix * c8) * 8;
        float v[8] = {0.f, 0.f, 0.f, 0.f, 0.f, 0.f, 0.f, 0.f};
        for (int k = 0; k < ksplit; ++k) {
            const float *p = ws + (size_t)k * pixels * C + pix * C + c;
            const float4 a = *reinterpret_cast<const float4 *>(p), b = *reinterpret_cast<const float4 *>(p + 4);
            v[0] += a.x; v[1] += a.y; v[2] += a.z; v[3] += a.w; v[4] += b.x; v[5] += b.y; v[6] += b.z; v[7] += b.w;
        }
        float amax = 0.f;
#pragma unroll
        for (int j = 0; j < 8; ++j) {
            if (bias) v[j] += bias[c + j];
            if (relu) v[j] = fmaxf(v[j], 0.f);
            amax = fmaxf(amax, fabsf(v[j]));
        }
        uint32_t hi[4], lo[4];
        if (split) {
#pragma unroll
            for (int k = 0; k < 4; ++k) {
                const __half2 h2 = __floats2half2_rn(v[2 * k], v[2 * k + 1]);
                const float2 hf = __half22float2(h2);
                const __half2 l2 = __floats2half2_rn(v[2 * k] - hf.x, v[2 * k + 1] - hf.y);
                hi[k] = *reinterpret_cast<const uint32_t *>(&h2);
                lo[k] = *reinterpret_cast<const uint32_t *>(&l2);
            }
            __half *o = static_cast<__half *>(out) + pix * 2 * C + c;
            *reinterpret_cast<uint4 *>(o) = make_uint4(hi[0], hi[1], hi[2], hi[3]);
            *reinterpret_cast<uint4 *>(o + C) = make_uint4(lo[0], lo[1], lo[2], lo[3]);
            if (amax > 65504.f) atomicAdd(ovf, 1u);
        } else {
#pragma unroll
            for (int k = 0; k < 4; ++k) {
                __nv_bfloat162 b2 = __floats2bfloat162_rn(v[2 * k], v[2 * k + 1]);
                hi[k] = *reinterpret_cast<uint32_t *>(&b2);
            }
            *reinterpret_cast<uint4 *>(static_cast<__nv_bfloat16 *>(out) + pix * C + c) = make_uint4(hi[0], hi[1], hi[2], hi[3]);
        }
    }
}
}
}

using namespace orp;

extern "C" int orp_tc_timing_collect(float *total_ms, int *launches, double *flops)
{
    if (!total_ms || !launches || !flops) return fail(ORP_EINVAL, "orp_tc_timing_collect: null");
    float sum = 0.f;
    for (int i = 0; i < g_tc_ev_used; ++i) {
        float ms = 0.f;
        ORP_CUDA(cudaEventSynchronize(g_tc_ev[i][1]));
        ORP_CUDA(cudaEventElapsedTime(&ms, g_tc_ev[i][0], g_tc_ev[i][1]));
        sum += ms;
        if (getenv("ORP_TC_TRACE")) {
            const TcTrace &t = g_tc_trace[i];
            fprintf(stderr, "tc[%3d] np=%d N=%d %4dx%-4d Cin=%4d Cout=%4d k=%d s=%d dcn=%d BN=%3d tiles=%5d grid=%3d  %8.1f us  %7.1f TFLOP/s\n",
                    i, t.nprob, t.N, t.H, t.W, t.Cin, t.Cout, t.K, t.stride, t.deform, t.BN, t.tiles, t.grid, ms * 1e3,
                    t.flops / (ms * 1e-3) / 1e12);
        }
    }
    *total_ms = sum; *launches = g_tc_ev_used; *flops = g_tc_flops;
    g_tc_ev_used = 0; g_tc_flops = 0.0;
    return ORP_OK;
}

extern "C" int orp_tc_last_plan(orp_tc_plan *out)
{
    if (!out) return fail(ORP_EINVAL, "orp_tc_last_plan: null");
    if (!g_tc_plan_set) return fail(ORP_EINVAL, "orp_tc_last_plan: no tensor-core convolution launched on this thread");
    *out = g_tc_plan;
    return ORP_OK;
}

extern "C" int orp_tc_plan_conv(int nprob, const orp_tc_problem *probs, const void *w, int Cout, int Cout_padded, int KH, int KW,
                                int Cin, int stride, int pad, const float *bias, int wscale_log2, int relu, int out_f32, int deform,
                                int split, int stem, int ksplit, int sms, orp_tc_plan *out)
{
    if (!out || sms < 1 || (stem != 0 && stem != 2)) return fail(ORP_EINVAL, "orp_tc_plan_conv: bad arguments");
    split = split ? 1 : 0;
    orp_tc_problem q;
    ConvDesc d;
    int rc = ORP_OK;
    if (stem == 2 || ksplit > 1) {
        if (nprob != 1 || !probs || deform || out_f32 || (stem == 2 && ksplit > 1))
            return fail(ORP_EINVAL, "orp_tc_plan_conv: the stem and split-K plan one problem with a 16-bit output");
        int Ho, Wo;
        rc = stem == 2 ? stem_desc(probs->x, probs->N, probs->H, probs->W, w, bias, relu, probs->out, split, wscale_log2, q, d)
                       : splitk_desc(probs, w, Cout, Cout_padded, KH, KW, Cin, stride, pad, split, wscale_log2, ksplit, probs->out, q,
                                     d, Ho, Wo);
    } else {
        d = ConvDesc{nprob, probs, w, Cout, Cout_padded, KH, KW, Cin, stride, pad, bias, relu, out_f32, deform, split, wscale_log2, 0, 1};
    }
    if (rc) return rc;
    ConvPlan pl;
    rc = plan_conv(d, sms, pl);
    if (rc) return rc;
    *out = pl.rep;
    return ORP_OK;
}

extern "C" int orp_conv2d_bf16(int nprob, const orp_tc_problem *probs, const void *w, int Cout, int Cout_padded, int KH,
                               int KW, int Cin, int stride, int pad, const float *bias, int relu, int out_f32,
                               int deform, void *stream)
{
    return conv2d_tc(ConvDesc{nprob, probs, w, Cout, Cout_padded, KH, KW, Cin, stride, pad, bias, relu, out_f32, deform, 0, 0, 0, 1},
                     stream);
}

extern "C" int orp_conv2d_f16x3(int nprob, const orp_tc_problem *probs, const void *w_split, int Cout, int Cout_padded, int KH,
                                int KW, int Cin, int stride, int pad, const float *bias, int wscale_log2, int relu,
                                int out_f32, int deform, void *stream)
{
    return conv2d_tc(ConvDesc{nprob, probs, w_split, Cout, Cout_padded, KH, KW, Cin, stride, pad, bias, relu, out_f32, deform, 1,
                              wscale_log2, 0, 1},
                     stream);
}

extern "C" int orp_stem_conv_s2d_f16x3(const void *x_s2d, int N, int H, int W, const void *w_split, const float *bias,
                                       int wscale_log2, int relu, void *out, void *stream)
{
    orp_tc_problem q;
    ConvDesc d;
    const int rc = stem_desc(x_s2d, N, H, W, w_split, bias, relu, out, 1, wscale_log2, q, d);
    return rc ? rc : conv2d_tc(d, stream);
}

extern "C" int orp_stem_conv_s2d_bf16(const void *x_s2d, int N, int H, int W, const void *w256, const float *bias, int relu,
                                      void *out, void *stream)
{
    orp_tc_problem q;
    ConvDesc d;
    const int rc = stem_desc(x_s2d, N, H, W, w256, bias, relu, out, 0, 0, q, d);
    return rc ? rc : conv2d_tc(d, stream);
}

extern "C" int orp_f16x3_overflow_count(unsigned int *count, int reset)
{
    if (!count) return fail(ORP_EINVAL, "f16x3_overflow_count: null");
    ORP_CUDA(cudaMemcpyFromSymbol(count, g_f16_overflow, sizeof(unsigned int)));
    if (reset) {
        const unsigned int z = 0;
        ORP_CUDA(cudaMemcpyToSymbol(g_f16_overflow, &z, sizeof(z)));
    }
    return ORP_OK;
}

extern "C" int orp_conv2d_tc_splitk(const orp_tc_problem *prob, const void *w, int Cout, int Cout_padded, int KH, int KW, int Cin,
                                    int stride, int pad, const float *bias, int f16x3, int wscale_log2, int relu, int ksplit,
                                    float *workspace, void *stream)
{
    orp_tc_problem q;
    ConvDesc d;
    int Ho = 0, Wo = 0;
    int rc = splitk_desc(prob, w, Cout, Cout_padded, KH, KW, Cin, stride, pad, f16x3, wscale_log2, ksplit, workspace, q, d, Ho, Wo);
    if (rc) return rc;
    rc = conv2d_tc(d, stream);
    if (rc) return rc;
    cudaStream_t st = static_cast<cudaStream_t>(stream);
    const size_t pixels = (size_t)prob->N * Ho * Wo;
    void *ovf = nullptr;
    ORP_CUDA(cudaGetSymbolAddress(&ovf, g_f16_overflow));
    splitk_finish_kernel<<<grid_for(pixels * (Cout / 8), 256), 256, 0, st>>>(workspace, ksplit, pixels, Cout, bias, relu, f16x3 ? 1 : 0, prob->out,
                                                                static_cast<unsigned int *>(ovf));
    ORP_LAUNCHED();
    if (prob->gn_stats) {
        if (Cout != 256) return fail(ORP_EINVAL, "conv2d_tc_splitk: gn_stats needs 256 output channels");
        return f16x3 ? orp_gn_stats_f16x3(prob->out, prob->N, Ho * Wo, 256, 32, prob->gn_stats, stream)
                     : orp_gn_stats_bf16(prob->out, prob->N, Ho * Wo, 256, 32, prob->gn_stats, stream);
    }
    return ORP_OK;
}
```

Before: 242.1.

## Pair deformable N tiles into BN=256 kernel with register-fragment epilogue

```diff
diff --git a/include/orp_b200.h b/include/orp_b200.h
--- a/include/orp_b200.h
+++ b/include/orp_b200.h
@@ -85,6 +85,7 @@
     int residual;
     int tma_epi, ncat, dcat, res_mma, b_resident, epi_merge, epi_bufs, gn_fused;
     int BW[5], BH[5], BI[5];
+    int n_pair;
 } orp_tc_plan;
 int orp_tc_last_plan(orp_tc_plan *out);
 
diff --git a/orientedreppoints_b200/_lib.py b/orientedreppoints_b200/_lib.py
--- a/orientedreppoints_b200/_lib.py
+++ b/orientedreppoints_b200/_lib.py
@@ -42,7 +42,7 @@
     _fields_ = [(k, _i) for k in ("BN", "stages", "grid", "num_tiles", "n_tiles_n", "ksplit", "nprob", "Cout", "Cout_padded",
                                   "split", "deform", "out_f32", "stem", "relu", "bias", "residual", "tma_epi", "ncat", "dcat",
                                   "res_mma", "b_resident", "epi_merge", "epi_bufs", "gn_fused")] + \
-              [(k, _i * 5) for k in ("BW", "BH", "BI")]
+              [(k, _i * 5) for k in ("BW", "BH", "BI")] + [("n_pair", _i)]
 
     def as_dict(self):
         d = {k: getattr(self, k) for k, _ in self._fields_}
diff --git a/orientedreppoints_b200/csrc/dense_tc.cu b/orientedreppoints_b200/csrc/dense_tc.cu
--- a/orientedreppoints_b200/csrc/dense_tc.cu
+++ b/orientedreppoints_b200/csrc/dense_tc.cu
@@ -165,6 +165,32 @@
 __device__ __forceinline__ float2 ffma2_rn(float2 a, float2 b, float2 c) { return make_float2(__fmaf_rn(a.x, b.x, c.x), __fmaf_rn(a.y, b.y, c.y)); }
 __device__ __forceinline__ float2 fadd2_rn(float2 a, float2 b) { return make_float2(__fadd_rn(a.x, b.x), __fadd_rn(a.y, b.y)); }
 
+__device__ __forceinline__ void split_sample(const uint4 (&u)[4][2], float4 wv, uint2 wh, uint32_t (&hi)[4], uint32_t (&lo)[4])
+{
+    const float2 wc[4] = {make_float2(wv.x, wv.x), make_float2(wv.y, wv.y), make_float2(wv.z, wv.z), make_float2(wv.w, wv.w)};
+    const __half2 wl[4] = {__low2half2(*reinterpret_cast<const __half2 *>(&wh.x)), __high2half2(*reinterpret_cast<const __half2 *>(&wh.x)),
+                           __low2half2(*reinterpret_cast<const __half2 *>(&wh.y)), __high2half2(*reinterpret_cast<const __half2 *>(&wh.y))};
+#pragma unroll
+    for (int k = 0; k < 4; ++k) {
+        float2 acc = make_float2(0.f, 0.f);
+        __half2 accl = __float2half2_rn(0.f);
+#pragma unroll
+        for (int c = 0; c < 4; ++c) {
+            const uint32_t uh = reinterpret_cast<const uint32_t *>(&u[c][0])[k];
+            const uint32_t ul = reinterpret_cast<const uint32_t *>(&u[c][1])[k];
+            acc = ffma2_rn(wc[c], __half22float2(*reinterpret_cast<const __half2 *>(&uh)), acc);
+            accl = __hfma2(wl[c], *reinterpret_cast<const __half2 *>(&ul), accl);
+        }
+        acc = fadd2_rn(acc, __half22float2(accl));
+        const __half2 h2 = __floats2half2_rn(acc.x, acc.y);
+        const float2 hf = __half22float2(h2);
+        const float2 rem = fadd2_rn(acc, make_float2(-hf.x, -hf.y));
+        const __half2 l2 = __floats2half2_rn(rem.x, rem.y);
+        hi[k] = *reinterpret_cast<const uint32_t *>(&h2);
+        lo[k] = *reinterpret_cast<const uint32_t *>(&l2);
+    }
+}
+
 __device__ __forceinline__ float act_fn(float v, int act)
 {
     if (act == 1) return fmaxf(v, 0.f);
@@ -254,7 +280,11 @@
 {
     return cat ? (b_resident ? 2 * kABytes : 2 * kABytes + 2 * BN * kBK * 2) : (b_resident ? kABytes : kABytes + BN * kBK * 2);
 }
-constexpr int dyn_smem_bytes(int stage_b, int stages, int extra) { return 1024 + kAccBytes + stages * stage_b + extra; }
+__host__ __device__ constexpr bool frag_epilogue(int BN, bool deform) { return deform && BN == 256; }
+constexpr int dyn_smem_bytes(int stage_b, int stages, int extra, bool frag_epi)
+{
+    return 1024 + (frag_epi ? 0 : kAccBytes) + stages * stage_b + extra;
+}
 
 template <int BN, int R>
 __device__ __forceinline__ void stage_acc(const float (&acc)[R], int pass, bool ncat, float *s_acc, int row0, int col0)
@@ -291,8 +321,21 @@
     if constexpr (G + 1 < NG) wgmma_cols64<NG, BF16, R, G + 1>(acc, da, db, accumulate);
 }
 
+template <int BN, bool BF16>
+__device__ __forceinline__ void wgmma_dcat(float (&acc)[BN / 2], uint64_t da, uint64_t db, uint32_t accumulate)
+{
+    if constexpr (BN == 256) {
+        wgmma_n<128, BF16>(acc_view<0, 64>(acc), da, db, accumulate);
+        wgmma_n<128, BF16>(acc_view<64, 64>(acc), da, db + (uint64_t)1024, accumulate);
+    } else {
+        wgmma_n<BN, BF16>(acc, da, db, accumulate);
+    }
+}
+
 constexpr int kProducerRegs = 40;
 constexpr int kConsumerRegs = 232;
+constexpr int kWideConsumerRegs = 160;
+constexpr int kWideProducerRegs = 96;
 
 template <int BN, bool OUT_F32, bool DEFORM, bool SPLIT, int WALK>
 __global__ void __launch_bounds__(DEFORM ? kConsumers + kDP : kConsumers + 128, 1)
@@ -307,13 +350,17 @@
     constexpr bool kCat = WALK == kWalkNcat || WALK == kWalkDcat;
     constexpr int kKMode = (SPLIT && !kCat) ? 1 : 0;
     static_assert(kConsumers + 128 == 384 && 2 * 128 * kConsumerRegs + 128 * kProducerRegs <= 65536, "register split");
+    constexpr bool kFragEpi = frag_epilogue(BN, DEFORM);
+    static_assert(!kFragEpi || (SPLIT && !OUT_F32), "fragment epilogue: deformable f16x3 with a TMA epilogue");
+    static_assert(kConsumers == 256 && kDP == 256 && 2 * 128 * kWideConsumerRegs + 2 * 128 * kWideProducerRegs <= 65536,
+                  "register split (wide deformable)");
     constexpr int kEpiThreads = kConsumers;
     constexpr int kWG = 2;
     constexpr int kAccN = (WALK == kWalkNcat) ? 2 * BN : BN;
     extern __shared__ __align__(1024) uint8_t smem_raw[];
     uint8_t *smem = reinterpret_cast<uint8_t *>((reinterpret_cast<uintptr_t>(smem_raw) + 1023) & ~uintptr_t(1023));
     float *s_acc = reinterpret_cast<float *>(smem);
-    smem += kAccBytes;
+    if constexpr (!kFragEpi) smem += kAccBytes;
     constexpr int kBBytes = BN * kBK * 2;
     const int kStageBytes = stage_bytes(BN, kCat, P.b_resident);
     const int kblocks_all = P.KH * P.KW * P.cin_blocks * kWTerms;
@@ -359,6 +406,7 @@
 
     if (warp < kConsumers / 32) {
         if constexpr (!DEFORM) setmaxnreg_inc<kConsumerRegs>();
+        if constexpr (kFragEpi) setmaxnreg_inc<kWideConsumerRegs>();
         const int cw = warp >> 2;
         const uint32_t a_off = (uint32_t)cw * 8192u;
         const bool leader = (threadIdx.x & 127) == 0;
@@ -388,6 +436,10 @@
                 held = next;
             };
             for (int kb = 0; kb < kblocks; ++kb, it.next()) {
+                if constexpr (kFragEpi) {
+                    wgmma_wait<0>();
+                    release(-1);
+                }
                 mbar_wait(&full[r.stage], r.phase);
                 const uint32_t sa = smem_u32(smem + (size_t)r.stage * kStageBytes);
                 const uint64_t da = make_desc_sw128(sa + a_off);
@@ -409,9 +461,9 @@
                     const uint64_t dbh = make_desc_sw128(sa + 2 * kABytes), dbl = make_desc_sw128(sa + 2 * kABytes + kBBytes);
 #pragma unroll
                     for (int k = 0; k < kBK / 16; ++k) {
-                        wgmma_n<BN, kBF16>(acc, dl + (uint64_t)(k * 2), dbh + (uint64_t)(k * 2), (kb | k) ? 1u : 0u);
-                        wgmma_n<BN, kBF16>(acc, da + (uint64_t)(k * 2), dbl + (uint64_t)(k * 2), 1u);
-                        wgmma_n<BN, kBF16>(acc, da + (uint64_t)(k * 2), dbh + (uint64_t)(k * 2), 1u);
+                        wgmma_dcat<BN, kBF16>(acc, dl + (uint64_t)(k * 2), dbh + (uint64_t)(k * 2), (kb | k) ? 1u : 0u);
+                        wgmma_dcat<BN, kBF16>(acc, da + (uint64_t)(k * 2), dbl + (uint64_t)(k * 2), 1u);
+                        wgmma_dcat<BN, kBF16>(acc, da + (uint64_t)(k * 2), dbh + (uint64_t)(k * 2), 1u);
                     }
                 } else {
                     const uint64_t db = make_desc_sw128(P.b_resident ? smem_u32(bres + (size_t)slab * kBBytes) : sa + kABytes);
@@ -472,7 +524,70 @@
             };
             size_t pix;
             const bool valid = row_pixel(rrow, pix);
-            if (OUT_F32) {
+            if constexpr (kFragEpi) {
+                const uint32_t obuf_u = smem_u32(stage_out);
+                const bool io = (et == 0);
+                if (nt != bias_nt) {
+                    bar_sync(bar_a, nthr);
+                    for (int c = et; c < BN; c += nthr) s_bias[c] = (P.bias && nt * BN + c < P.Cout) ? P.bias[nt * BN + c] : 0.f;
+                    bias_nt = nt;
+                }
+                size_t pix_r[2];
+                const bool valid_r[2] = {row_pixel(frow, pix_r[0]), row_pixel(frow + 8, pix_r[1])};
+                float amax[2][2] = {{0.f, 0.f}, {0.f, 0.f}};
+#pragma unroll
+                for (int pass = 0; pass < 2 * (BN / 64); ++pass) {
+                    const int half = pass >> 1, oterm = pass & 1;
+                    if (io) {
+                        if (P.epi_bufs == 2) asm volatile("cp.async.bulk.wait_group.read 1;" ::: "memory");
+                        else asm volatile("cp.async.bulk.wait_group.read 0;" ::: "memory");
+                    }
+                    bar_sync(bar_a, nthr);
+                    const uint32_t obase = obuf_u + (uint32_t)ob * 16384u;
+#pragma unroll
+                    for (int i = 0; i < 8; ++i) {
+                        const int g = half * 8 + i;
+                        const float2 bv = *reinterpret_cast<const float2 *>(&s_bias[g * 8 + fcol]);
+#pragma unroll
+                        for (int hr = 0; hr < 2; ++hr) {
+                            const int row = frow + 8 * hr;
+                            float f0 = acc[4 * g + 2 * hr], f1 = acc[4 * g + 2 * hr + 1];
+                            f0 *= P.oscale; f1 *= P.oscale;
+                            f0 += bv.x; f1 += bv.y;
+                            if (P.relu) { f0 = fmaxf(f0, 0.f); f1 = fmaxf(f1, 0.f); }
+                            if (oterm == 0) amax[hr][i >> 2] = fmaxf(fmaxf(amax[hr][i >> 2], fabsf(f0)), fabsf(f1));
+                            const __half2 h2 = __floats2half2_rn(f0, f1);
+                            uint32_t v = *reinterpret_cast<const uint32_t *>(&h2);
+                            if (oterm) {
+                                const float2 hf = __half22float2(h2);
+                                const __half2 l2 = __floats2half2_rn(f0 - hf.x, f1 - hf.y);
+                                v = *reinterpret_cast<const uint32_t *>(&l2);
+                            }
+                            const uint32_t at = obase + (uint32_t)row * 128u + ((uint32_t)(i ^ (row & 7)) << 4) + (uint32_t)fcol * 2u;
+                            asm volatile("st.shared.b32 [%0], %1;" ::"r"(at), "r"(v) : "memory");
+                        }
+                    }
+                    asm volatile("fence.proxy.async.shared::cta;" ::: "memory");
+                    bar_sync(bar_b, nthr);
+                    if (io) {
+                        asm volatile(
+                            "cp.async.bulk.tensor.5d.global.shared::cta.bulk_group [%0, {%2, %3, %4, %5, %6}], [%1];"
+                            ::"l"(&P.tmOut[pi]), "r"(obase), "r"(nt * BN + half * 64), "r"(oterm),
+                              "r"(wb * pr.BW), "r"(hb * pr.BH), "r"(ib * pr.BI) : "memory");
+                        asm volatile("cp.async.bulk.commit_group;" ::: "memory");
+                    }
+                    if (++ob == P.epi_bufs) ob = 0;
+                }
+#pragma unroll
+                for (int hr = 0; hr < 2; ++hr)
+#pragma unroll
+                    for (int hc = 0; hc < 2; ++hc) {
+                        float m = amax[hr][hc];
+                        m = fmaxf(m, __shfl_xor_sync(0xffffffffu, m, 1));
+                        m = fmaxf(m, __shfl_xor_sync(0xffffffffu, m, 2));
+                        if ((lane & 3) == 0 && valid_r[hr] && m > 65504.f) atomicAdd(P.ovf, 1u);
+                    }
+            } else if (OUT_F32) {
 #pragma unroll 1
                 for (int pass = 0; pass < BN / HC; ++pass) {
                 bar_sync(bar_a, nthr);
@@ -773,6 +888,7 @@
         __shared__ float4 s_w[2][128];
         __shared__ uint2 s_wh[2][128];
         __shared__ int4 s_o[2][128];
+        if constexpr (kFragEpi) setmaxnreg_dec<kWideProducerRegs>();
         const int pt = threadIdx.x - kConsumers;
         auto load_b = [&](int stage, int tap, int cb, int nt) {
             uint8_t *sb = smem + (size_t)stage * kStageBytes + (P.dcat ? 2 * kABytes : kABytes);
@@ -787,21 +903,17 @@
             int pi, wb, hb, ib, nt;
             decode_tile(P, tile, pi, wb, hb, ib, nt);
             const Problem &pr = P.prob[pi];
-            bool valid = false;
-            int w = 0, h = 0, n = 0;
-            if (pt < 128) {
-                const int iw = pt & (pr.BW - 1), ih = (pt >> pr.lbw) & (pr.BH - 1), ii = pt >> (pr.lbw + pr.lbh);
-                w = wb * pr.BW + iw; h = hb * pr.BH + ih; n = ib * pr.BI + ii;
-                valid = (w < pr.Wo) && (h < pr.Ho) && (n < pr.N);
-            }
             const int taps = P.KH * P.KW;
-            const size_t opix = ((size_t)(valid ? n : 0) * pr.Ho + (valid ? h : 0)) * pr.Wo + (valid ? w : 0);
-            const float *offp = pr.offset + opix * (2 * taps);
-            const float *mskp = pr.mask ? pr.mask + opix * taps : nullptr;
-            const int cpp = P.Cin * (P.split ? 2 : 1);
-            const int img0 = (valid ? n : 0) * pr.H * pr.W * cpp;
             for (int tap = 0; tap < taps; ++tap) {
                 if (pt < 128) {
+                    const int iw = pt & (pr.BW - 1), ih = (pt >> pr.lbw) & (pr.BH - 1), ii = pt >> (pr.lbw + pr.lbh);
+                    const int w = wb * pr.BW + iw, h = hb * pr.BH + ih, n = ib * pr.BI + ii;
+                    const bool valid = (w < pr.Wo) && (h < pr.Ho) && (n < pr.N);
+                    const size_t opix = ((size_t)(valid ? n : 0) * pr.Ho + (valid ? h : 0)) * pr.Wo + (valid ? w : 0);
+                    const float *offp = pr.offset + opix * (2 * taps);
+                    const float *mskp = pr.mask ? pr.mask + opix * taps : nullptr;
+                    const int cpp = P.Cin * (SPLIT ? 2 : 1);
+                    const int img0 = (valid ? n : 0) * pr.H * pr.W * cpp;
                     const int kh = tap / P.KW, kw = tap - kh * P.KW;
                     float4 wv = make_float4(0.f, 0.f, 0.f, 0.f);
                     int4 ov = make_int4(img0, img0, img0, img0);
@@ -831,7 +943,7 @@
                 }
                 asm volatile("bar.sync 2, %0;" ::"n"(kDP) : "memory");
                 for (int cb = 0; cb < P.cin_blocks; ++cb) {
-                    if (!P.split) {
+                    if constexpr (!SPLIT) {
                         mbar_wait(&empty[r.stage], r.phase ^ 1);
                         if (pt == 0) load_b(r.stage, tap, cb, nt);
                         uint8_t *sa = smem + (size_t)r.stage * kStageBytes;
@@ -874,67 +986,69 @@
                         r.next();
                     } else {
                         const __half *xh = reinterpret_cast<const __half *>(pr.x);
-                        uint32_t phi[kDItems][4], plo[kDItems][4];
-#pragma unroll
-                        for (int i2 = 0; i2 < 2; ++i2) {
-                            uint4 u[kDRound][4][2];
-#pragma unroll
-                            for (int i1 = 0; i1 < kDRound; ++i1) {
-                                const int item = pt + (i2 * kDRound + i1) * kDP, row = item >> 3, c16 = item & 7;
-                                const int4 ov = s_o[tb][row];
-                                const int co = cb * kBK + c16 * 8;
-                                const int oo[4] = {ov.x, ov.y, ov.z, ov.w};
-#pragma unroll
-                                for (int c = 0; c < 4; ++c) {
-                                    u[i1][c][0] = *reinterpret_cast<const uint4 *>(xh + oo[c] + co);
-                                    u[i1][c][1] = *reinterpret_cast<const uint4 *>(xh + oo[c] + P.Cin + co);
+                        auto load_item = [&](int it, uint4 (&u)[4][2]) {
+                            const int item = pt + it * kDP, row = item >> 3, c16 = item & 7;
+                            const int4 ov = s_o[tb][row];
+                            const int co = cb * kBK + c16 * 8;
+                            const int oo[4] = {ov.x, ov.y, ov.z, ov.w};
+#pragma unroll
+                            for (int c = 0; c < 4; ++c) {
+                                u[c][0] = *reinterpret_cast<const uint4 *>(xh + oo[c] + co);
+                                u[c][1] = *reinterpret_cast<const uint4 *>(xh + oo[c] + P.Cin + co);
+                            }
+                        };
+                        auto item_at = [&](int it) {
+                            const int item = pt + it * kDP, row = item >> 3, c16 = item & 7;
+                            return (uint32_t)(row * 128 + ((c16 ^ (row & 7)) << 4));
+                        };
+                        if constexpr (!kFragEpi) {
+                            uint32_t phi[kDItems][4], plo[kDItems][4];
+#pragma unroll
+                            for (int i2 = 0; i2 < kDItems / kDRound; ++i2) {
+                                uint4 u[kDRound][4][2];
+#pragma unroll
+                                for (int i1 = 0; i1 < kDRound; ++i1) load_item(i2 * kDRound + i1, u[i1]);
+#pragma unroll
+                                for (int i1 = 0; i1 < kDRound; ++i1) {
+                                    const int it = i2 * kDRound + i1, row = (pt + it * kDP) >> 3;
+                                    split_sample(u[i1], s_w[tb][row], s_wh[tb][row], phi[it], plo[it]);
                                 }
                             }
-#pragma unroll
-                            for (int i1 = 0; i1 < kDRound; ++i1) {
-                                const int it = i2 * kDRound + i1, item = pt + it * kDP, row = item >> 3;
-                                const float4 wv = s_w[tb][row];
-                                const uint2 wh = s_wh[tb][row];
-                                const float2 wc[4] = {make_float2(wv.x, wv.x), make_float2(wv.y, wv.y), make_float2(wv.z, wv.z), make_float2(wv.w, wv.w)};
-                                const __half2 wl[4] = {__low2half2(*reinterpret_cast<const __half2 *>(&wh.x)), __high2half2(*reinterpret_cast<const __half2 *>(&wh.x)),
-                                                       __low2half2(*reinterpret_cast<const __half2 *>(&wh.y)), __high2half2(*reinterpret_cast<const __half2 *>(&wh.y))};
-#pragma unroll
-                                for (int k = 0; k < 4; ++k) {
-                                    float2 acc = make_float2(0.f, 0.f);
-                                    __half2 accl = __float2half2_rn(0.f);
-#pragma unroll
-                                    for (int c = 0; c < 4; ++c) {
-                                        const uint32_t uh = reinterpret_cast<const uint32_t *>(&u[i1][c][0])[k];
-                                        const uint32_t ul = reinterpret_cast<const uint32_t *>(&u[i1][c][1])[k];
-                                        acc = ffma2_rn(wc[c], __half22float2(*reinterpret_cast<const __half2 *>(&uh)), acc);
-                                        accl = __hfma2(wl[c], *reinterpret_cast<const __half2 *>(&ul), accl);
-                                    }
-                                    acc = fadd2_rn(acc, __half22float2(accl));
-                                    const __half2 h2 = __floats2half2_rn(acc.x, acc.y);
-                                    const float2 hf = __half22float2(h2);
-                                    const float2 rem = fadd2_rn(acc, make_float2(-hf.x, -hf.y));
-                                    const __half2 l2 = __floats2half2_rn(rem.x, rem.y);
-                                    phi[it][k] = *reinterpret_cast<const uint32_t *>(&h2);
-                                    plo[it][k] = *reinterpret_cast<const uint32_t *>(&l2);
-                                }
-                            }
-                        }
-                        {
                             mbar_wait(&empty[r.stage], r.phase ^ 1);
                             if (pt == 0) load_b(r.stage, tap, cb, nt);
                             uint8_t *sa = smem + (size_t)r.stage * kStageBytes;
 #pragma unroll
                             for (int it = 0; it < kDItems; ++it) {
-                                const int item = pt + it * kDP, row = item >> 3, c16 = item & 7;
-                                const size_t at = (size_t)row * 128 + ((c16 ^ (row & 7)) << 4);
+                                const uint32_t at = item_at(it);
                                 *reinterpret_cast<uint4 *>(sa + at) = make_uint4(phi[it][0], phi[it][1], phi[it][2], phi[it][3]);
                                 *reinterpret_cast<uint4 *>(sa + kABytes + at) = make_uint4(plo[it][0], plo[it][1], plo[it][2], plo[it][3]);
                             }
-                            asm volatile("fence.proxy.async.shared::cta;" ::: "memory");
-                            __syncwarp();
-                            if ((pt & 31) == 0) mbar_arrive(&full[r.stage]);
-                            r.next();
+                        } else {
+                            const uint32_t sa = smem_u32(smem + (size_t)r.stage * kStageBytes);
+#pragma unroll
+                            for (int i2 = 0; i2 < kDItems / kDRound; ++i2) {
+                                uint4 u[kDRound][4][2];
+#pragma unroll
+                                for (int i1 = 0; i1 < kDRound; ++i1) load_item(i2 * kDRound + i1, u[i1]);
+                                if (i2 == 0) {
+                                    mbar_wait(&empty[r.stage], r.phase ^ 1);
+                                    if (pt == 0) load_b(r.stage, tap, cb, nt);
+                                }
+#pragma unroll
+                                for (int i1 = 0; i1 < kDRound; ++i1) {
+                                    const int it = i2 * kDRound + i1, row = (pt + it * kDP) >> 3;
+                                    uint32_t hi[4], lo[4];
+                                    split_sample(u[i1], s_w[tb][row], s_wh[tb][row], hi, lo);
+                                    const uint32_t at = sa + item_at(it);
+                                    sts128(at, make_uint4(hi[0], hi[1], hi[2], hi[3]));
+                                    sts128(at + kABytes, make_uint4(lo[0], lo[1], lo[2], lo[3]));
+                                }
+                            }
                         }
+                        asm volatile("fence.proxy.async.shared::cta;" ::: "memory");
+                        __syncwarp();
+                        if ((pt & 31) == 0) mbar_arrive(&full[r.stage]);
+                        r.next();
                     }
                 }
                 tb ^= 1;
@@ -992,6 +1106,7 @@
     orp_tc_plan rep;
     Problem prob[kMaxProb];
     int num_m_tiles;
+    int kbn;
     int extra_bytes;
 };
 
@@ -1035,6 +1150,8 @@
     if (d.deform && BN > 128) BN = 128;
     const int cin_blocks = (d.Cin + kBK - 1) / kBK;
     const int n_tiles_n = d.Cout_padded / BN;
+    const int n_pair = (d.deform && d.split && !d.out_f32 && d.Cout % 8 == 0 && d.relu != 2 && BN == 128 && n_tiles_n % 2 == 0) ? 2 : 1;
+    const int kbn = BN * n_pair;
     int mt = 0;
     for (int i = 0; i < nprob; ++i) {
         const orp_tc_problem &q = probs[i];
@@ -1061,7 +1178,8 @@
     const int tma_epi = (!d.out_f32 && ((d.Cout % 64 == 0) || (d.split && d.Cout % 8 == 0)) && BN >= 64) ? 1 : 0;
     if (d.split && !d.out_f32 && !tma_epi) return fail(ORP_EINVAL, "conv2d_f16x3: 16-bit outputs need Cout % 8 == 0 and weights padded to a multiple of 64 rows");
     if (d.split && d.out_f32 && any_res) return fail(ORP_EINVAL, "conv2d_f16x3: fp32 outputs take an fp32 residual only");
-    bool want_gn = false, gn_ok = tma_epi && d.Cout == 256 && !d.bias && !d.relu;
+    const bool frag_epi = frag_epilogue(kbn, d.deform != 0);
+    bool want_gn = false, gn_ok = tma_epi && d.Cout == 256 && !d.bias && !d.relu && !frag_epi;
     for (int i = 0; i < nprob; ++i) {
         want_gn = want_gn || (probs[i].gn_stats != nullptr);
         if (pl.prob[i].BW * pl.prob[i].BH < 32) gn_ok = false;
@@ -1069,7 +1187,7 @@
     const int gn_fused = (want_gn && gn_ok) ? 1 : 0;
     const bool mem_bound = any_res || (d.KH * d.KW * (d.Cin / kBK) <= 8);
     int epi_bufs = mem_bound ? 2 : 1;
-    const int epi_merge = (d.split && tma_epi && (mem_bound || d.stem == 2)) ? 1 : 0;
+    const int epi_merge = (d.split && tma_epi && !frag_epi && (mem_bound || d.stem == 2)) ? 1 : 0;
     const int dcat = (d.split && d.deform) ? 1 : 0;
     const int ncat = (d.split && tma_epi && BN <= 128 && !d.deform && !any_res) ? 1 : 0;
     const int res_mma = (tma_epi && any_res) ? 1 : 0;
@@ -1080,17 +1198,17 @@
     }
     const int slab_bytes = d.KH * d.KW * T * cin_blocks * BN * kBK * 2;
     int b_resident = (!d.deform && ksplit == 1 && slab_bytes <= 72 * 1024) ? 1 : 0;
-    int grid = num_tiles < sms ? num_tiles : sms;
+    int grid = num_tiles / n_pair < sms ? num_tiles / n_pair : sms;
     if (b_resident && grid >= n_tiles_n) grid -= grid % n_tiles_n;
     else if (b_resident) b_resident = 0;
     int stage_b = 0, extra = 0, stages = 0;
     for (;;) {
-        stage_b = stage_bytes(BN, ncat || dcat, b_resident);
+        stage_b = stage_bytes(kbn, ncat || dcat, b_resident);
         const int hc = BN < 64 ? BN : 64;
         int staging = d.out_f32 ? 0 : 128 * (hc * 2 + 16);
         if (tma_epi) staging = epi_bufs * (epi_merge ? 32768 : 16384);
         extra = (res_mma ? 8192 : 0) + (b_resident ? slab_bytes : 0) + staging;
-        stages = (kSmemPerBlock - (d.deform ? kStaticSmemDeform : kStaticSmemPlain) - dyn_smem_bytes(stage_b, 0, extra)) / stage_b;
+        stages = (kSmemPerBlock - (d.deform ? kStaticSmemDeform : kStaticSmemPlain) - dyn_smem_bytes(stage_b, 0, extra, frag_epi)) / stage_b;
         if (stages >= 3) break;
         if (epi_bufs == 2) { epi_bufs = 1; continue; }
         if (b_resident) { b_resident = 0; continue; }
@@ -1101,6 +1219,7 @@
     if (d.deform && stages > 3) stages = 3;
 
     pl.num_m_tiles = mt;
+    pl.kbn = kbn;
     pl.extra_bytes = extra;
     orp_tc_plan &r = pl.rep;
     r.BN = BN; r.stages = stages; r.grid = grid; r.num_tiles = num_tiles; r.n_tiles_n = n_tiles_n;
@@ -1113,7 +1232,7 @@
         r.BW[i] = pl.prob[i].BW; r.BH[i] = pl.prob[i].BH; r.BI[i] = pl.prob[i].BI;
     }
     r.tma_epi = tma_epi; r.ncat = ncat; r.dcat = dcat; r.res_mma = res_mma; r.b_resident = b_resident;
-    r.epi_merge = epi_merge; r.epi_bufs = epi_bufs; r.gn_fused = gn_fused;
+    r.epi_merge = epi_merge; r.epi_bufs = epi_bufs; r.gn_fused = gn_fused; r.n_pair = n_pair;
     return ORP_OK;
 }
 
@@ -1130,7 +1249,7 @@
         ORP_CUDA(cudaGetSymbolAddress(&ovf, g_f16_overflow));
         P.ovf = static_cast<unsigned int *>(ovf);
     }
-    P.n_tiles_n = pl.rep.n_tiles_n;
+    P.n_tiles_n = pl.rep.n_tiles_n / pl.rep.n_pair;
     P.fd_ntn.set((uint32_t)P.n_tiles_n);
     for (int i = 0; i < d.nprob; ++i) {
         const orp_tc_problem &q = d.probs[i];
@@ -1140,7 +1259,7 @@
         pr.x = static_cast<const __nv_bfloat16 *>(q.x); pr.offset = q.offset; pr.gn_stats = q.gn_stats; pr.mask = q.mask;
     }
     P.num_m_tiles = pl.num_m_tiles;
-    P.num_tiles = pl.rep.num_tiles;
+    P.num_tiles = pl.rep.num_tiles / pl.rep.n_pair;
     P.ksplit = d.ksplit;
     P.fd_ks.set((uint32_t)d.ksplit);
     P.ks_stride = (long long)P.prob[0].N * P.prob[0].Ho * P.prob[0].Wo * d.Cout;
@@ -1180,7 +1299,7 @@
         const cuuint64_t K = (cuuint64_t)d.KH * d.KW * T * P.cin_blocks * kBK;
         cuuint64_t gdim[2] = {K, (cuuint64_t)d.Cout_padded};
         cuuint64_t gstr[1] = {K * 2};
-        cuuint32_t box[2] = {(cuuint32_t)kBK, (cuuint32_t)pl.rep.BN};
+        cuuint32_t box[2] = {(cuuint32_t)kBK, (cuuint32_t)pl.kbn};
         cuuint32_t estr[2] = {1, 1};
         CUresult r = enc(&P.tmB, dt16, 2, const_cast<void *>(d.w), gdim, gstr, box, estr,
                          CU_TENSOR_MAP_INTERLEAVE_NONE, CU_TENSOR_MAP_SWIZZLE_128B, CU_TENSOR_MAP_L2_PROMOTION_L2_256B,
@@ -1230,7 +1349,7 @@
 int launch_tc(const TcParams &P, int stages, int grid, cudaStream_t st, int extra_bytes)
 {
     constexpr bool kCat = WALK == kWalkNcat || WALK == kWalkDcat;
-    const int smem = dyn_smem_bytes(stage_bytes(BN, kCat, P.b_resident), stages, extra_bytes);
+    const int smem = dyn_smem_bytes(stage_bytes(BN, kCat, P.b_resident), stages, extra_bytes, frag_epilogue(BN, DEFORM));
     auto kern = conv_tc_kernel<BN, OUT_F32, DEFORM, SPLIT, WALK>;
     static int smem_max = -1;
     if (smem_max < 0) {
@@ -1286,8 +1405,14 @@
 {
     if constexpr (DEFORM) {
         if (P.dcat != P.split || P.ncat || P.res_mma) return fail(ORP_EINVAL, "conv2d_tc: deformable plan outside dcat == split");
-        return P.split ? launch_tc<BN, OUT_F32, true, true, kWalkDcat>(P, stages, grid, st, extra_bytes)
-                       : launch_tc<BN, OUT_F32, true, false, kWalkK>(P, stages, grid, st, extra_bytes);
+        if constexpr (frag_epilogue(BN, true)) {
+            if (!P.split || OUT_F32 || !P.tma_epi || P.epi_merge || P.gn_fused || P.relu == 2)
+                return fail(ORP_EINVAL, "conv2d_tc: deformable N-tile pair outside f16x3 with an unmerged TMA epilogue and no GELU");
+            return launch_tc<BN, false, true, true, kWalkDcat>(P, stages, grid, st, extra_bytes);
+        } else {
+            return P.split ? launch_tc<BN, OUT_F32, true, true, kWalkDcat>(P, stages, grid, st, extra_bytes)
+                           : launch_tc<BN, OUT_F32, true, false, kWalkK>(P, stages, grid, st, extra_bytes);
+        }
     } else {
         if (P.ncat && P.res_mma) return fail(ORP_EINVAL, "conv2d_tc: ncat plan with a residual");
         if (P.ncat) {
@@ -1311,9 +1436,9 @@
 int launch_bn(const TcParams &P, const ConvPlan &pl, cudaStream_t st)
 {
     const int s = pl.rep.stages, g = pl.rep.grid, e = pl.extra_bytes;
-    switch (pl.rep.BN) {
+    switch (pl.kbn) {
     case 256:
-        if constexpr (!DEFORM) return launch_plan<256, OUT_F32, false>(P, s, g, st, e);
+        if constexpr (!DEFORM || !OUT_F32) return launch_plan<256, OUT_F32, DEFORM>(P, s, g, st, e);
         break;
     case 128: return launch_plan<128, OUT_F32, DEFORM>(P, s, g, st, e);
     case 64: return launch_plan<64, OUT_F32, DEFORM>(P, s, g, st, e);
```

Result: faster. 255.6, median of 6 (+5.6%).
